# Aatricks/LightDiffusion-Next

Measured on AMD Instinct MI355X. Metric: sampler it/s (UNet steps/sec) SD1.5 1024x1024 bs=1 bf16, higher is better.
Workload: dtype bf16

## Files before the change

### include/ldx.h

```cpp
#ifndef LDX_H
#define LDX_H
#include <stdint.h>
#ifdef __cplusplus
extern "C" {
#endif

#define LDX_OK 0
#define LDX_EINVAL (-1)
#define LDX_EMISSING (-2)
#define LDX_EHIP (-3)
#define LDX_ESTATE (-4)

#define LDX_BF16 0
#define LDX_F16 1
#define LDX_F32 2

typedef struct ldx_engine ldx_engine;

typedef struct ldx_unet_config {
    int32_t compute_dtype;
    int32_t in_channels;
    int32_t out_channels;
    int32_t model_channels;
    int32_t num_levels;
// ... 33 lines not shown
    int32_t d_ff;
    int32_t num_layers;
    int32_t num_heads;
    int32_t vocab_size;
} ldx_t5_config;

typedef struct ldx_esrgan_config {
    int32_t compute_dtype;
    int32_t in_nc;
    int32_t out_nc;
    int32_t nf;
    int32_t gc;
    int32_t num_blocks;
    int32_t num_upscale;
} ldx_esrgan_config;

typedef struct ldx_flux_config {
    int32_t compute_dtype;
    int32_t in_channels;
    int32_t vec_in_dim;
    int32_t context_in_dim;
    int32_t hidden_size;
    int32_t mlp_hidden;
    int32_t num_heads;
    int32_t depth;
    int32_t depth_single;
    int32_t guidance_embed;
} ldx_flux_config;

const char* ldx_version(void);
const char* ldx_last_error(void);
int ldx_create(const ldx_unet_config* cfg, int device, ldx_engine** out);
void ldx_destroy(ldx_engine* e);
int ldx_load_tensor(ldx_engine* e, const char* key, const void* data, int dtype, const int64_t* shape, int ndim);
int ldx_set_tables(ldx_engine* e, const float* log_sigmas, int n, const float* temb, int temb_dim);
int ldx_finalize(ldx_engine* e);

int ldx_unet_denoise(ldx_engine* e, const float* x_nchw, const float* sigma, const float* ctx,
                     int B2, int h, int w, int M, float* out_nchw, void* stream);
int ldx_unet_denoise_concat(ldx_engine* e, const float* x_nchw, const float* sigma, const float* ctx, const float* c_concat, int cc_channels,
                            int B2, int h, int w, int M, float* out_nchw, void* stream);
int ldx_unet_denoise_cfg(ldx_engine* e, const float* x_nchw, float sigma, const float* ctx,
                         int B, int h, int w, int M, float* out_nchw, void* stream);
int ldx_unet_denoise_cfg_t(ldx_engine* e, const float* x_nchw, float sigma, int t_index, const float* ctx,
                           int B, int h, int w, int M, float* out_nchw, void* stream);
int ldx_unet_denoise_t(ldx_engine* e, const float* x_nchw, const float* sigma, const float* t_index, const float* ctx,
                       int B2, int h, int w, int M, float* out_nchw, void* stream);
int ldx_unet_timestep(ldx_engine* e, const float* sigma, int n, int32_t* t_out, void* stream);
int ldx_unet_context_cache(ldx_engine* e, int enable);
int ldx_unet_forward(ldx_engine* e, const float* x_nchw, const float* timesteps, const float* ctx,
                     int B2, int h, int w, int M, float* out_nchw, void* stream);
int ldx_plan_info(ldx_engine* e, int64_t* n_launches, double* flops, int64_t* arena_bytes);
int ldx_unet_cfg_share(ldx_engine* e, int enable);
int ldx_plan_flops(ldx_engine* e, double* executed, double* shared);
int ldx_profile(ldx_engine* e, int enable, int reset);
int ldx_profile_report(ldx_engine* e, char* buf, int64_t cap);
int ldx_set_graph_mode(ldx_engine* e, int enable);
int ldx_graph_stats(ldx_engine* e, int64_t* captures, int64_t* replays);
int ldx_reload_env(void);

int ldx_vae_create(const ldx_vae_config* cfg, int device, ldx_engine** out);
int ldx_vae_decode(ldx_engine* e, const float* z_nchw, int B, int h, int w, float* out_nhwc, void* stream);
int ldx_vae_encode(ldx_engine* e, const float* pixels_nhwc, int B, int H, int W, float* moments_nchw, void* stream);
int ldx_clip_create(const ldx_clip_config* cfg, int device, ldx_engine** out);
int ldx_clip_encode(ldx_engine* e, const int32_t* ids, int B, int T, int inter_layer,
                    float* out_last, float* out_inter, void* stream);
int ldx_clip_pooled(ldx_engine* e, const float* last, const int32_t* ids, int B, int T, int eos_token_id,
                    float* out_pooled, void* stream);
int ldx_clip_set_extra_embeddings(ldx_engine* e, const float* rows_host, int n);

int ldx_esrgan_create(const ldx_esrgan_config* cfg, int device, ldx_engine** out);
int ldx_esrgan_forward(ldx_engine* e, const float* pixels_nhwc, int B, int H, int W, float* out_nhwc, void* stream);
int ldx_tile_blend(const float* tile, int th, int tw, float* out, float* div, int H, int W, int C, int y0, int x0, int feather, void* stream);
int ldx_tile_finish(float* out, const float* div, int64_t n, int clamp01, void* stream);

int ldx_flux_fbcache(ldx_engine* e, float residual_diff_threshold);
int ldx_flux_fbcache_stats(ldx_engine* e, int64_t* hits, int64_t* misses);
int ldx_flux_set_fp8(ldx_engine* e, int enable);

int ldx_t5_create(const ldx_t5_config* cfg, int device, ldx_engine** out);
int ldx_t5_encode(ldx_engine* e, const int32_t* ids, int B, int L, const float* bias, float* out, void* stream);

int ldx_flux_create(const ldx_flux_config* cfg, int device, ldx_engine** out);
int ldx_flux_forward(ldx_engine* e, const float* x, const float* sigma, const float* ctx, const float* y,
                     const float* guidance, const float* pe_cos, const float* pe_sin,
                     int B, int h, int w, int Lt, int denoise, float* out, void* stream);

int ldx_sampler_step(int kind, float* x, const float* den_uncond, const float* den_cond, float* denoised_out,
                     int64_t n, float cfg, float c0, float c1, void* stream);
int ldx_bislerp_pass(const float* in, float* out, int N, int C, int H, int W, int axis, int new_len,
                     const int32_t* c1, const int32_t* c2, const float* ratios, void* stream);
int ldx_bilinear(const float* in, float* out, int planes, int hin, int win, int hout, int wout, void* stream);

int ldx_op_convert(const float* in_f32, void* out_16, int64_t n, int dtype, int to_f32, void* stream);
int ldx_op_gemm(const void* A, int lda, const void* W, int M, int N, int K, const float* bias,
                const float* rowvec, int rowvec_ld, int rows_per_batch, int geglu,
                const void* R, int ldr, void* C, int ldc, float* Cf, int ldcf, int dtype, void* stream);
int ldx_op_layernorm_mx(const void* X, int ldx, int rows, int C, float eps, const float* gamma, const float* beta,
                        void* Y8, int ldy8, void* S8, int s8_ld, int dtype, void* stream);
int ldx_op_qk_norm_rope_mx(const void* QKV, int ld, int rows, int L, int H, const float* qscale, const float* kscale, const float* cosT, const float* sinT, float eps,
                           void* Q8, void* K8, int ld8, void* SQ, void* SK, int s_ld, int dtype, void* stream);
int ldx_op_mx_vt_quant(const void* V, int ldv, int B, int H, int L, void* V8T, void* SV, int Lp, int dtype, void* stream);
int ldx_op_attention_fp8(const void* Q8, int ldq8, const void* SQ, int sq_ld, const void* K8, int ldk8, const void* SK, int sk_ld, const void* V8T, const void* SV, int Lp,
                         void* O, int ldo, void* O8, int ldo8, void* SO, int so_ld, int B, int H, int Nq, int Mk, float scale, int dtype, void* stream);
int ldx_op_attention_mx(const void* Q, int ldq, const void* K, int ldk, const void* V, int ldv, void* O8, int ldo8, void* SO, int so_ld,
                        int B, int H, int Nq, int Mk, float scale, int dtype, void* stream);
int ldx_op_mx_quant(const void* X, int ldx, int rows, int K, void* Y, int ldy, void* scales, int scales_ld, int dtype, void* stream);
int ldx_op_gemm_mx(const void* A8, int lda, const void* SA, int sa_ld, const void* W8, const void* SW, int sw_ld, int M, int N, int K,
                   const float* bias, int act, const void* R, int ldr, void* C, int ldc, float* Cf, int ldcf,
                   void* C8, int ldc8, void* SC, int sc_ld, int dtype, void* stream);
int ldx_op_gemm2(const void* A1, int lda1, const void* W1, int M1, int N1, int K1, const float* bias1, void* C1, int ldc1,
                 const void* A2, int lda2, const void* W2, int M2, int N2, int K2, const float* bias2, void* C2, int ldc2, int dtype, void* stream);
int ldx_op_gemm2_mx(const void* A1, int lda1, const void* SA1, int sa_ld1, const void* W1, const void* SW1, int sw_ld1, int M1, int N1, int K1,
                    const float* bias1, void* C1, int ldc1,
                    const void* A2, int lda2, const void* SA2, int sa_ld2, const void* W2, const void* SW2, int sw_ld2, int M2, int N2, int K2,
                    const float* bias2, void* C2, int ldc2, int dtype, void* stream);
int ldx_op_gemm_pick(int M, int N, int K, int mode, int geglu, int splitk, int f8, int c8, int ln_fold,
                     int Cin, int Hin, int Win, int Hout, int Wout, int stride, int M2, int N2, int K2,
                     int gn_hw, int gn_groups, int gn_max_chunks, int32_t* out);
int ldx_op_attn_pick(int B, int H, int Nq, int Mk, int D, int causal, int bias, int o8, int ldq, int ldk, int ldv, int ldo, int knorm_ws, int32_t* out);
int ldx_op_conv3x3(const void* X, int ldx, const void* W, int B, int Hin, int Win, int Cin, int Cout,
                   int stride, int Hout, int Wout, int resize_to_out, const float* bias,
                   const float* rowvec, int rowvec_ld, const void* R, int ldr, void* Y, int ldy,
                   int dtype, void* stream);
int ldx_op_conv3x3_skip(const void* X, int ldx, const void* X2, int ldx2, int Cin2, const void* W, int B, int H, int Wd, int Cin, int Cout,
                        const float* bias, void* Y, int ldy, int dtype, void* stream);
int ldx_op_groupnorm(const void* X, int ldx, void* Y, int ldy, int B, int HW, int C, int G, float eps, int silu,
                     const float* gamma, const float* beta, float* workspace, int dtype, void* stream);
int64_t ldx_op_groupnorm_workspace_floats(int B, int G);
int ldx_op_layernorm(const void* X, int ldx, void* Y, int ldy, int rows, int C, float eps,
                     const float* gamma, const float* beta, int dtype, void* stream);
int ldx_op_attention(const void* Q, int ldq, const void* K, int ldk, const void* V, int ldv, void* O, int ldo,
                     int B, int H, int Nq, int Mk, int D, float scale, int causal, int dtype, void* stream);
int ldx_op_xattn_block(void* H, int ldh, int64_t M, int N, int C, int heads, const float* ln_gamma, const float* ln_beta, float eps,
                       const void* Wq, const void* Wo, const float* bo, const void* K, int ldk, const void* V, int ldv, int Mk,
                       float scale, int dtype, void* stream);
int ldx_op_ff_block(void* H, int ldh, int64_t M, int C, int inner, const float* ln_gamma, const float* ln_beta, float eps,
                    const void* W1, const float* b1, const void* W2, const float* b2, int dtype, void* stream);
int ldx_op_rowgemm(const void* X, int ldx, void* Y, int ldy, int64_t M, int N, int K, const void* W, const float* bias, const void* R, int ldr,
                   int pro, const float* gamma, const float* beta, float eps, const float* partial, int nchunk, int HW, int dtype, void* stream);
int ldx_op_attention_bias(const void* Q, int ldq, const void* K, int ldk, const void* V, int ldv, void* O, int ldo,
                          int B, int H, int Nq, int Mk, int D, float scale, const float* bias, int bias_ld,
                          int64_t bias_head_stride, int dtype, void* stream);
int ldx_op_skinny(const float* x, int ldx, const void* W, const float* bias, float* out, int ldo,
                  int M, int N, int K, int in_act, int out_act, int dtype, void* stream);

#ifdef __cplusplus
}
#endif
#endif
```

### lightdiffusion-next_amd/csrc/attn_pipe.hip

```cpp
#include <stdlib.h>
#include <math.h>
#include <type_traits>
#include <utility>
#include "ldx_device.h"
#include "ldx_kernels.h"
#include "attn_pipe_common.h"

namespace ldx {

template <typename T>
__global__ __launch_bounds__(256) void attn_knorm_kernel(const AttnArgs p) {
    const int lane = threadIdx.x & 63, nblk = (p.Mk + 63) >> 6;
    const long w = (long)blockIdx.x * 4 + (threadIdx.x >> 6);
    if (w >= (long)p.B * p.H * nblk) return;
    const int blk = (int)(w % nblk), hb = (int)(w / nblk), h = hb % p.H, b = hb / p.H;
    const int key = blk * 64 + lane;
    float ss = 0.f;
    if (key < p.Mk) {
        const T* kp = (const T*)p.K + ((long)b * p.Mk + key) * p.ldk + h * p.D;
        for (int ch = 0; ch < p.D / 8; ++ch) {
            float f[8]; unpack8<T>(*(const uint4*)(kp + ch * 8), f);
#pragma unroll
            for (int e = 0; e < 8; ++e) ss = fmaf(f[e], f[e], ss);
        }
// ... 261 lines not shown
            });
        };
        if constexpr (KB) {
            if (__builtin_amdgcn_ballot_w64(ap_max2(bm0, bm1) > thr) != 0) {
                asm volatile("s_nop 15\n\ts_nop 15" ::: "memory");
                ap_for(ap_range<0, 8>(), [&](auto M) __attribute__((always_inline)) { maxblk(M, sn); });
                bm0 = bmax(0); bm1 = bmax(1);
                if (__builtin_amdgcn_ballot_w64(ap_max2(bm0, bm1) > thr) != 0) raise_reference();
            }
        } else {
            if (__builtin_amdgcn_ballot_w64(ap_max2(bm0, bm1) > thr) != 0) raise_reference();
        }
    };
    const unsigned klast = (unsigned)(nblk - 1) * kstep, vlast = (unsigned)(nblk - 1) * vstep;
    unsigned kofs = min(4u * kstep, klast), vofs = min(2u * vstep, vlast);
    for (int t = 0; t < nblk; t += 2) {
        slot(t, sA, sB, pA, pB, vfA, vfB, rsA, rsB, ap_ic<0>{}, kofs, vofs);
        kofs = min(kofs + kstep, klast); vofs = min(vofs + vstep, vlast);
        slot(t + 1, sB, sA, pB, pA, vfB, vfA, rsB, rsA, ap_ic<1>{}, kofs, vofs);
        kofs = min(kofs + kstep, klast); vofs = min(vofs + vstep, vlast);
    }
    ap_for(ap_range<0, 16>(), [&](auto J) __attribute__((always_inline)) { pv1(J, pA, vfA); });
    asm volatile("s_nop 15\n\ts_nop 15\n\ts_nop 15" ::: "memory");

#pragma unroll
    for (int qt = 0; qt < 2; ++qt) {
        const float mine = (h2 == 0) ? o[qt][1][4] : 0.f;
        auto sw = __builtin_amdgcn_permlane32_swap(__float_as_uint(mine), __float_as_uint(mine), false, false);
        const float l = __uint_as_float(sw[0]) + __uint_as_float(sw[1]);
        const float inv = (l > 0.f) ? 1.0f / l : 0.f;
        const int q = q0 + qt * 32 + l31;
#pragma unroll
        for (int dt = 0; dt < 2; ++dt)
#pragma unroll
            for (int rq = 0; rq < 4; ++rq) {
                const int d = dt * 32 + 8 * rq + 4 * h2;
                if (d < D)
                    *(uint2*)(Op + (long)q * p.ldo + d) = pack4<T>(o[qt][dt][4 * rq] * inv, o[qt][dt][4 * rq + 1] * inv, o[qt][dt][4 * rq + 2] * inv, o[qt][dt][4 * rq + 3] * inv);
            }
    }
}


void launch_attn_knorm(const AttnArgs& a, DType dt, hipStream_t s) {
    const long waves = (long)a.B * a.H * ((a.Mk + 63) / 64);
    if (dt == DT_BF16) hipLaunchKernelGGL((attn_knorm_kernel<__bf16>), dim3((unsigned)((waves + 3) / 4)), dim3(256), 0, s, a);
    else hipLaunchKernelGGL((attn_knorm_kernel<_Float16>), dim3((unsigned)((waves + 3) / 4)), dim3(256), 0, s, a);
}

template <typename T, int ABL = 0>
static void launch_attn40p(const AttnArgs& a, const AttnPick& p, hipStream_t s, float thr) {
    if (p.knorm && ABL == 0) {
        const long waves = (long)a.B * a.H * ((a.Mk + 63) / 64);
        hipLaunchKernelGGL((attn_knorm_kernel<T>), dim3((unsigned)((waves + 3) / 4)), dim3(256), 0, s, a);
        hipLaunchKernelGGL((attn40p_kernel<T, ABL, true>), dim3(p.grid), dim3(p.block), p.lds, s, a, thr);
    } else {
        hipLaunchKernelGGL((attn40p_kernel<T, ABL, false>), dim3(p.grid), dim3(p.block), p.lds, s, a, thr);
    }
}

void launch_attn_pipe(const AttnArgs& a, const AttnPick& p, DType dt, hipStream_t s) {
    const bool ov = p.thr == p.thr;
#ifdef LDX_ATTN_ABLATE
    if (const char* e = getenv("LDX_ATTN_PIPE_ABL")) {
        const float thr = ApT<__bf16>::thr;
        switch (atoi(e)) {
            case 1: launch_attn40p<__bf16, 1>(a, p, s, thr); return;
            case 2: launch_attn40p<__bf16, 2>(a, p, s, thr); return;
            case 8: launch_attn40p<__bf16, 8>(a, p, s, thr); return;
            case 16: launch_attn40p<__bf16, 16>(a, p, s, thr); return;
            case 32: launch_attn40p<__bf16, 32>(a, p, s, thr); return;
            case 9: launch_attn40p<__bf16, 9>(a, p, s, thr); return;
            case 25: launch_attn40p<__bf16, 25>(a, p, s, thr); return;
            case 27: launch_attn40p<__bf16, 27>(a, p, s, thr); return;
            case 59: launch_attn40p<__bf16, 59>(a, p, s, thr); return;
            default: break;
        }
    }
#endif
    if (dt == DT_BF16) launch_attn40p<__bf16>(a, p, s, ov ? p.thr : ApT<__bf16>::thr);
    else launch_attn40p<_Float16>(a, p, s, ov ? fminf(p.thr, ApT<_Float16>::thr) : ApT<_Float16>::thr);
}

}
```

### lightdiffusion-next_amd/csrc/attn_pipe128.hip

```cpp
#include <stdlib.h>
#include <math.h>
#include "ldx_device.h"
#include "ldx_kernels.h"
#include "attn_pipe_common.h"

namespace ldx {

template <typename T> __device__ __forceinline__ int ap128_half_a(float sa, float c, float nm, float& x, float px, float py) {
    int r;
    if constexpr (std::is_same<T, __bf16>::value) asm("v_fma_f32 %1, %2, %3, %4\n\tv_exp_f32 %1, %1\n\tv_cvt_pk_bf16_f32 %0, %5, %6" : "=&v"(r), "=&v"(x) : "v"(sa), "s"(c), "v"(nm), "v"(px), "v"(py));
    else asm("v_fma_f32 %1, %2, %3, %4\n\tv_exp_f32 %1, %1\n\tv_cvt_pk_f16_f32 %0, %5, %6" : "=&v"(r), "=&v"(x) : "v"(sa), "s"(c), "v"(nm), "v"(px), "v"(py));
    return r;
}
template <typename T> __device__ __forceinline__ void ap128_half_b(float sb, float c, float nm, float& y, float& l, int r, int ones) {
    if constexpr (std::is_same<T, __bf16>::value) asm("v_fma_f32 %0, %2, %3, %4\n\tv_exp_f32 %0, %0\n\tv_dot2_f32_bf16 %1, %5, %6, %1" : "=&v"(y), "+v"(l) : "v"(sb), "s"(c), "v"(nm), "v"(r), "s"(ones));
    else asm("v_fma_f32 %0, %2, %3, %4\n\tv_exp_f32 %0, %0\n\tv_dot2_f32_f16 %1, %5, %6, %1" : "=&v"(y), "+v"(l) : "v"(sb), "s"(c), "v"(nm), "v"(r), "s"(ones));
}
__device__ __forceinline__ void ap128_exp1(float s, float c, float nm, float& x) {
    asm("v_fma_f32 %0, %1, %2, %3\n\tv_exp_f32 %0, %0" : "=&v"(x) : "v"(s), "s"(c), "v"(nm));
}
template <typename T> __device__ __forceinline__ void ap128_sacc0(f32x16& d, ap_i32x4 a, ap_i32x4 b) {
    if constexpr (std::is_same<T, __bf16>::value) asm volatile(AP_BF16 " %0, %1, %2, 0" : "=&v"(d) : "v"(a), "a"(b));
    else asm volatile(AP_F16 " %0, %1, %2, 0" : "=&v"(d) : "v"(a), "a"(b));
}
// ... 271 lines not shown
    constexpr int EROW = 272, EROW8 = 144;
    char* ep = smem + wave * (64 * EROW);
#pragma unroll
    for (int qt = 0; qt < 2; ++qt) {
        auto sw = __builtin_amdgcn_permlane32_swap(__float_as_uint(lsum[qt]), __float_as_uint(lsum[qt]), false, false);
        const float l = __uint_as_float(sw[0]) + __uint_as_float(sw[1]);
        const float inv = (l > 0.f) ? 1.0f / l : 0.f;
        const int q = q0 + qt * 32 + l31;
        if (p.O8) {
            uint32_t sc = 0;
#pragma unroll
            for (int dt = 0; dt < 4; ++dt) {
                float v[16], amax = 0.f;
#pragma unroll
                for (int r = 0; r < 16; ++r) { v[r] = to_f32(from_f32<T>(o[qt][dt][r] * inv)); amax = fmaxf(amax, fabsf(v[r])); }
                auto am = __builtin_amdgcn_permlane32_swap(__float_as_uint(amax), __float_as_uint(amax), false, false);
                amax = fmaxf(__uint_as_float(am[0]), __uint_as_float(am[1]));
                const int e = mx_scale_e8m0(amax);
                const float is = mx_inv_scale(e);
                sc |= (uint32_t)e << (8 * dt);
#pragma unroll
                for (int rq = 0; rq < 4; ++rq)
                    *(uint32_t*)(ep + (qt * 32 + l31) * EROW8 + dt * 32 + 8 * rq + 4 * h2) = mx_pack4(v[4 * rq] * is, v[4 * rq + 1] * is, v[4 * rq + 2] * is, v[4 * rq + 3] * is);
            }
            if (h2 == 0) p.SO[(long)h * p.so_ld + (long)b * p.Nq + q] = sc;
            continue;
        }
#pragma unroll
        for (int dt = 0; dt < 4; ++dt)
#pragma unroll
            for (int rq = 0; rq < 4; ++rq)
                *(uint2*)(ep + (qt * 32 + l31) * EROW + (dt * 32 + 8 * rq + 4 * h2) * 2) = pack4<T>(o[qt][dt][4 * rq] * inv, o[qt][dt][4 * rq + 1] * inv, o[qt][dt][4 * rq + 2] * inv, o[qt][dt][4 * rq + 3] * inv);
    }
    asm volatile("s_waitcnt lgkmcnt(0)" ::: "memory");
    if (p.O8) {
        char* o8 = (char*)p.O8 + ((long)b * p.Nq + q0) * p.ldo8 + h * 128;
#pragma unroll
        for (int i = 0; i < 8; ++i) {
            const int row = i * 8 + (lane >> 3), ch = lane & 7;
            *(uint4*)(o8 + (long)row * p.ldo8 + ch * 16) = *(const uint4*)(ep + row * EROW8 + ch * 16);
        }
    } else {
#pragma unroll
        for (int i = 0; i < 16; ++i) {
            const int row = i * 4 + (lane >> 4), ch = lane & 15;
            *(uint4*)(Op + (long)(q0 + row) * p.ldo + ch * 8) = *(const uint4*)(ep + row * EROW + ch * 16);
        }
    }
}

template <typename T, int ABL = 0>
static void launch_attn128p(const AttnArgs& a, const AttnPick& p, hipStream_t s, float thr) {
    if (p.knorm && ABL == 0) {
        launch_attn_knorm(a, std::is_same<T, __bf16>::value ? DT_BF16 : DT_F16, s);
        static DevOnce once;
        set_dyn_lds(once, (const void*)attn128p_kernel<T, ABL, true>, p.lds);
        hipLaunchKernelGGL((attn128p_kernel<T, ABL, true>), dim3(p.grid), dim3(p.block), p.lds, s, a, thr);
    } else {
        static DevOnce once;
        set_dyn_lds(once, (const void*)attn128p_kernel<T, ABL, false>, p.lds);
        hipLaunchKernelGGL((attn128p_kernel<T, ABL, false>), dim3(p.grid), dim3(p.block), p.lds, s, a, thr);
    }
}

void launch_attn_pipe128(const AttnArgs& a, const AttnPick& p, DType dt, hipStream_t s) {
    const bool ov = p.thr == p.thr;
#ifdef LDX_ATTN_ABLATE
    if (const char* e = getenv("LDX_ATTN_PIPE_ABL")) {
        const float thr = ApT<__bf16>::thr;
        switch (atoi(e)) {
            case 1: launch_attn128p<__bf16, 1>(a, p, s, thr); return;
            case 2: launch_attn128p<__bf16, 2>(a, p, s, thr); return;
            case 4: launch_attn128p<__bf16, 4>(a, p, s, thr); return;
            case 8: launch_attn128p<__bf16, 8>(a, p, s, thr); return;
            case 16: launch_attn128p<__bf16, 16>(a, p, s, thr); return;
            case 32: launch_attn128p<__bf16, 32>(a, p, s, thr); return;
            case 34: launch_attn128p<__bf16, 34>(a, p, s, thr); return;
            case 24: launch_attn128p<__bf16, 24>(a, p, s, thr); return;
            case 58: launch_attn128p<__bf16, 58>(a, p, s, thr); return;
            case 62: launch_attn128p<__bf16, 62>(a, p, s, thr); return;
            default: break;
        }
    }
#endif
    if (dt == DT_BF16) launch_attn128p<__bf16>(a, p, s, ov ? p.thr : ApT<__bf16>::thr);
    else launch_attn128p<_Float16>(a, p, s, ov ? fminf(p.thr, ApT<_Float16>::thr) : ApT<_Float16>::thr);
}

}
```

### lightdiffusion-next_amd/csrc/capi.cpp

```cpp
#include <cstring>
#include <mutex>
#include <new>

#include "engine.h"

using namespace ldx;

struct ldx_engine { Engine* impl; };

#define GUARD_BEGIN try {
#define GUARD_END                                                                  \
    }                                                                              \
    catch (const std::bad_alloc&) { set_error("out of host memory"); return LDX_EINVAL; } \
    catch (const std::exception& ex) { set_error(std::string("internal error: ") + ex.what()); return LDX_EINVAL; }

static int check_device(int device) {
    int n = 0;
    if (hipGetDeviceCount(&n) != hipSuccess || n <= 0) { set_error("no HIP device available (libldx has no CPU fallback)"); return LDX_EHIP; }
    if (device < 0 || device >= n) { set_error("device ordinal out of range"); return LDX_EINVAL; }
    return LDX_OK;
}
static inline DType dtype_of(int d) { return d == LDX_F16 ? DT_F16 : DT_BF16; }
static int check_launch(const char* what) {
    hipError_t e = hipGetLastError();
// ... 223 lines not shown
}
int ldx_unet_denoise_cfg(ldx_engine* e, const float* x, float sigma, const float* ctx, int B, int h, int w, int M, float* out, void* stream) {
    GUARD_BEGIN
    if (!e) { set_error("null engine"); return LDX_EINVAL; }
    if (e->impl->kind != KIND_UNET) { set_error("ldx_unet_denoise_cfg: not a UNet engine"); return LDX_ESTATE; }
    return e->impl->run_cfg(x, sigma, ctx, B, h, w, M, out, (hipStream_t)stream);
    GUARD_END
}
int ldx_unet_denoise_cfg_t(ldx_engine* e, const float* x, float sigma, int t_index, const float* ctx, int B, int h, int w, int M, float* out, void* stream) {
    GUARD_BEGIN
    if (!e) { set_error("null engine"); return LDX_EINVAL; }
    if (e->impl->kind != KIND_UNET) { set_error("ldx_unet_denoise_cfg_t: not a UNet engine"); return LDX_ESTATE; }
    return e->impl->run_cfg(x, sigma, ctx, B, h, w, M, out, (hipStream_t)stream, t_index < 0 ? -1 : t_index);
    GUARD_END
}
int ldx_unet_denoise_t(ldx_engine* e, const float* x, const float* sigma, const float* t_index, const float* ctx, int B2, int h, int w, int M, float* out, void* stream) {
    GUARD_BEGIN
    if (!e) { set_error("null engine"); return LDX_EINVAL; }
    if (e->impl->kind != KIND_UNET) { set_error("ldx_unet_denoise_t: not a UNet engine"); return LDX_ESTATE; }
    if (!t_index) { set_error("ldx_unet_denoise_t: t_index is null (use ldx_unet_denoise)"); return LDX_EINVAL; }
    return e->impl->run(x, sigma, ctx, B2, h, w, M, out, true, (hipStream_t)stream, 0, nullptr, 0, t_index);
    GUARD_END
}
int ldx_unet_timestep(ldx_engine* e, const float* sigma, int n, int32_t* t_out, void* stream) {
    GUARD_BEGIN
    if (!e) { set_error("null engine"); return LDX_EINVAL; }
    return e->impl->timestep_lookup(sigma, n, (int*)t_out, (hipStream_t)stream);
    GUARD_END
}
int ldx_unet_forward(ldx_engine* e, const float* x, const float* t, const float* ctx, int B2, int h, int w, int M, float* out, void* stream) {
    GUARD_BEGIN
    if (!e) { set_error("null engine"); return LDX_EINVAL; }
    if (e->impl->kind != KIND_UNET) { set_error("ldx_unet_forward: not a UNet engine"); return LDX_ESTATE; }
    return e->impl->run(x, t, ctx, B2, h, w, M, out, false, (hipStream_t)stream);
    GUARD_END
}
int ldx_plan_info(ldx_engine* e, int64_t* n_launches, double* flops, int64_t* arena_bytes) {
    if (!e) { set_error("null engine"); return LDX_EINVAL; }
    if (n_launches) *n_launches = e->impl->n_launches();
    if (flops) *flops = e->impl->algorithmic_flops();
    if (arena_bytes) *arena_bytes = (int64_t)e->impl->cur.arena_cap;
    return LDX_OK;
}
int ldx_plan_flops(ldx_engine* e, double* executed, double* shared) {
    if (!e) { set_error("null engine"); return LDX_EINVAL; }
    if (executed) *executed = e->impl->steady_flops();
    if (shared) *shared = e->impl->cur.flops_shared;
    return LDX_OK;
}
int ldx_unet_cfg_share(ldx_engine* e, int enable) {
    if (!e) { set_error("null engine"); return LDX_EINVAL; }
    if (e->impl->kind != KIND_UNET) { set_error("ldx_unet_cfg_share: not a UNet engine"); return LDX_ESTATE; }
    e->impl->cfg_share = enable < 0 ? 0 : (enable > 2 ? 2 : enable);
    return LDX_OK;
}
int ldx_profile(ldx_engine* e, int enable, int reset) {
    if (!e) { set_error("null engine"); return LDX_EINVAL; }
    e->impl->profiling = enable != 0;
    e->impl->prof_detail = enable == 2;
    if (reset) e->impl->prof.clear();
    return LDX_OK;
}
int ldx_profile_report(ldx_engine* e, char* buf, int64_t cap) {
    if (!e || !buf || cap <= 0) { set_error("ldx_profile_report: bad argument"); return LDX_EINVAL; }
    const std::string s = e->impl->profile_json();
    if ((int64_t)s.size() + 1 > cap) { set_error("ldx_profile_report: buffer too small"); return LDX_EINVAL; }
    memcpy(buf, s.c_str(), s.size() + 1);
    return LDX_OK;
}
int ldx_set_graph_mode(ldx_engine* e, int enable) {
    if (!e) { set_error("null engine"); return LDX_EINVAL; }
    e->impl->graph_mode = enable != 0;
    return LDX_OK;
}
int ldx_unet_context_cache(ldx_engine* e, int enable) {
    if (!e) { set_error("null engine"); return LDX_EINVAL; }
    if (e->impl->kind != KIND_UNET) { set_error("ldx_unet_context_cache: not a UNet engine"); return LDX_ESTATE; }
    return e->impl->set_context_cache(enable);
}
int ldx_reload_env(void) {
    reload_dispatch_env();
    return LDX_OK;
}
int ldx_graph_stats(ldx_engine* e, int64_t* captures, int64_t* replays) {
    if (!e || !captures || !replays) { set_error("ldx_graph_stats: bad argument"); return LDX_EINVAL; }
    *captures = e->impl->n_graph_captures; *replays = e->impl->n_graph_replays;
    return LDX_OK;
}

int ldx_sampler_step(int kind, float* x, const float* du, const float* dc, float* dout, int64_t n, float cfg, float c0, float c1, void* stream) {
    if (!x || !du || !dc || n < 0 || (kind < 0 || kind > 3)) { set_error("ldx_sampler_step: bad argument"); return LDX_EINVAL; }
    if (kind == 2 && !dout) { set_error("ldx_sampler_step: kind 2 (CFG combine only) needs denoised_out"); return LDX_EINVAL; }
    if (kind == 0 && c0 == 0.f) { set_error("ldx_sampler_step: kind 0 (Euler) divides by c0 = sigma_hat, which must be non-zero"); return LDX_EINVAL; }
    StepArgs a{x, du, dc, dout, (size_t)n, cfg, kind, c0, c1};
    launch_sampler_step(a, (hipStream_t)stream);
    return check_launch("ldx_sampler_step");
}
int ldx_bislerp_pass(const float* in, float* out, int N, int C, int H, int W, int axis, int new_len,
                     const int32_t* c1, const int32_t* c2, const float* ratios, void* stream) {
    if (!in || !out || !c1 || !c2 || !ratios || N <= 0 || C <= 0 || C > 16 || H <= 0 || W <= 0 || new_len <= 0 || (axis != 0 && axis != 1)) {
        set_error("ldx_bislerp_pass: bad argument (C <= 16, axis 0|1)"); return LDX_EINVAL; }
    launch_bislerp_pass(in, out, N, C, H, W, axis, new_len, (const int*)c1, (const int*)c2, ratios, (hipStream_t)stream);
    return check_launch("ldx_bislerp_pass");
}
int ldx_vae_encode(ldx_engine* e, const float* pixels_nhwc, int B, int H, int W, float* moments_nchw, void* stream) {
    GUARD_BEGIN
// ... 206 lines not shown
    launch_groupnorm(a, dtype_of(dtype), (hipStream_t)stream);
    return check_launch("ldx_op_groupnorm");
}
int ldx_op_layernorm(const void* X, int ldx_, void* Y, int ldy, int rows, int C, float eps, const float* gamma, const float* beta, int dtype, void* stream) {
    if (!X || !Y || !gamma || !beta || C % 8 || C > 4096) { set_error("ldx_op_layernorm: bad argument (C % 8, C <= 4096)"); return LDX_EINVAL; }
    LayerNormArgs a{X, ldx_, Y, ldy, rows, C, eps, gamma, beta};
    launch_layernorm(a, dtype_of(dtype), (hipStream_t)stream);
    return check_launch("ldx_op_layernorm");
}
int ldx_op_attention(const void* Q, int ldq, const void* K, int ldk, const void* V, int ldv, void* O, int ldo, int B, int H, int Nq, int Mk, int D,
                     float scale, int causal, int dtype, void* stream) {
    if (!Q || !K || !V || !O || D % 8 || (D > 160 && D != 512) || D <= 0 || ldq % 8 || ldk % 8 || ldv % 8 || ldo % 4 || Mk <= 0) { set_error("ldx_op_attention: bad argument (D % 8, D <= 160 or D == 512)"); return LDX_EINVAL; }
    AttnArgs a{Q, ldq, K, ldk, V, ldv, O, ldo, B, H, Nq, Mk, D, scale, causal, nullptr, 0, 0};
    const AttnPick p = attn_pick(a);
    if (D == 512 && p.family != AF_ATTN512) { set_error("ldx_op_attention: D = 512 without a mask only (attn512.hip)"); return LDX_EINVAL; }
    if (p.nsplit_want > 1) {
        a.nsplit = p.nsplit_want;
        a.split_ws = op_workspace(attn512_ws_floats(a, a.nsplit));
        if (!a.split_ws) { set_error("attention split workspace allocation failed"); return LDX_EHIP; }
    }
    if (attn_pipe_ok(a)) a.knorm_ws = op_workspace((size_t)B * H * ((Mk + 63) / 64));
    launch_attention(a, dtype_of(dtype), (hipStream_t)stream);
    return check_launch("ldx_op_attention");
}
int ldx_op_xattn_block(void* H, int ldh, int64_t M, int N, int C, int heads, const float* ln_gamma, const float* ln_beta, float eps,
                       const void* Wq, const void* Wo, const float* bo, const void* K, int ldk, const void* V, int ldv, int Mk,
                       float scale, int dtype, void* stream) {
    XAttnArgs a{};
    a.H = H; a.ldh = ldh; a.M = (long)M; a.N = N; a.C = C; a.heads = heads; a.ln_g = ln_gamma; a.ln_b = ln_beta; a.eps = eps;
    a.Wq = Wq; a.Wo = Wo; a.bo = bo; a.K = K; a.ldk = ldk; a.V = V; a.ldv = ldv; a.Mk = Mk; a.scale = scale;
    if (!H || !ln_gamma || !ln_beta || !Wq || !Wo || !K || !V || M <= 0 || N <= 0 || ldh < C || !xattn_block_ok(a)) {
        set_error("ldx_op_xattn_block: shape not taken by the fused kernel (C = 320, 8 heads, Mk <= 80, N % 128 == 0, M % N == 0)"); return LDX_EINVAL; }
    launch_xattn_block(a, dtype_of(dtype), (hipStream_t)stream);
    return check_launch("ldx_op_xattn_block");
}
int ldx_op_ff_block(void* H, int ldh, int64_t M, int C, int inner, const float* ln_gamma, const float* ln_beta, float eps,
                    const void* W1, const float* b1, const void* W2, const float* b2, int dtype, void* stream) {
    FFBlockArgs a{};
    a.H = H; a.ldh = ldh; a.M = (long)M; a.C = C; a.inner = inner; a.ln_g = ln_gamma; a.ln_b = ln_beta; a.eps = eps; a.W1 = W1; a.b1 = b1; a.W2 = W2; a.b2 = b2;
    if (!H || !ln_gamma || !ln_beta || !W1 || !b1 || !W2 || M <= 0 || ldh < C || !ff_block_ok(a)) {
        set_error("ldx_op_ff_block: shape not taken by the fused kernel (C = 320, inner = 1280)"); return LDX_EINVAL; }
    launch_ff_block(a, dtype_of(dtype), (hipStream_t)stream);
    return check_launch("ldx_op_ff_block");
}
int ldx_op_rowgemm(const void* X, int ldx_, void* Y, int ldy, int64_t M, int N, int K, const void* W, const float* bias, const void* R, int ldr,
                   int pro, const float* gamma, const float* beta, float eps, const float* partial, int nchunk, int HW, int dtype, void* stream) {
    RowGemmArgs a{};
    a.X = X; a.ldx = ldx_; a.Y = Y; a.ldy = ldy; a.M = (long)M; a.N = N; a.K = K; a.W = W; a.bias = bias; a.R = R; a.ldr = ldr;
    a.pro = pro; a.g = gamma; a.b = beta; a.eps = eps; a.partial = partial; a.nchunk = nchunk; a.HW = HW; a.G = 32;
    if (!X || !Y || !W || ldx_ < K || ldy < N || !rowgemm_ok(a)) { set_error("ldx_op_rowgemm: shape not taken (K = 320 or 640, N a multiple of K, pro 0..2, GroupNorm: HW % (40960 / K) == 0, nchunk <= 256)"); return LDX_EINVAL; }
    launch_rowgemm(a, dtype_of(dtype), (hipStream_t)stream);
    return check_launch("ldx_op_rowgemm");
}
int ldx_op_attention_bias(const void* Q, int ldq, const void* K, int ldk, const void* V, int ldv, void* O, int ldo, int B, int H, int Nq, int Mk, int D,
                          float scale, const float* bias, int bias_ld, int64_t bias_head_stride, int dtype, void* stream) {
    if (!Q || !K || !V || !O || !bias || D % 8 || D > 160 || D <= 0 || ldq % 8 || ldk % 8 || ldv % 8 || ldo % 4 || Mk <= 0 || bias_ld % 4 ||
        bias_ld < ((Mk + 63) / 64) * 64 || bias_head_stride % 4) {
        set_error("ldx_op_attention_bias: bad argument (bias_ld >= Mk rounded up to 64, multiples of 4)"); return LDX_EINVAL; }
    AttnArgs a{Q, ldq, K, ldk, V, ldv, O, ldo, B, H, Nq, Mk, D, scale, 0, bias, bias_ld, (long)bias_head_stride};
    launch_attention(a, dtype_of(dtype), (hipStream_t)stream);
    return check_launch("ldx_op_attention_bias");
}
int ldx_op_skinny(const float* x, int ldx_, const void* W, const float* bias, float* out, int ldo, int M, int N, int K, int in_act, int out_act, int dtype, void* stream) {
    if (!x || !W || !out || K % 8) { set_error("ldx_op_skinny: bad argument"); return LDX_EINVAL; }
    SkinnyArgs a{x, ldx_, W, bias, out, ldo, M, N, K, in_act, out_act};
    launch_skinny(a, dtype_of(dtype), (hipStream_t)stream);
    return check_launch("ldx_op_skinny");
}

}
```

### lightdiffusion-next_amd/csrc/engine.cpp

```cpp
#include "engine.h"

#include <algorithm>
#include <cmath>
#include <cstdio>
#include <cstring>
#include <thread>

namespace ldx {

thread_local std::string g_last_error;
void set_error(const std::string& s) { g_last_error = s; }
int launch_status() {
    const hipError_t e = hipGetLastError();
    if (e == hipSuccess) return LDX_OK;
    set_error(std::string("kernel launch: ") + hipGetErrorString(e));
    return LDX_EHIP;
}

#define HIP_OK(expr)                                                                         \
    do {                                                                                     \
        hipError_t _e = (expr);                                                              \
        if (_e != hipSuccess) {                                                              \
            set_error(std::string(#expr) + ": " + hipGetErrorString(_e));                    \
            return LDX_EHIP;                                                                 \
// ... 547 lines not shown
        GemmArgs& g = cur.ops[i - 1].g;
        GroupNormArgs& n = cur.ops[i].gn;
        if (g.C != n.X || g.ldc != n.ldx || g.N != n.C || (long)g.M != (long)n.B * n.HW) continue;
        const int nchunk = gemm_gn_fuse(g, n.HW, n.G, gn_ws_rows);
        if (!nchunk) continue;
        g.gn_partial = n.partial;
        n.stats_chunks = nchunk;
        cur.ops[i].bytes = 2.0 * 2.0 * (double)n.B * n.HW * n.C;
        snprintf(cur.ops[i].klabel, sizeof(cur.ops[i].klabel), "gn_apply(fused stats)");
    }
}
bool Engine::rowblock_fills_chip(long workgroups) const {
    static const long min_wg = getenv("LDX_ROWBLOCK_MINWG") ? atol(getenv("LDX_ROWBLOCK_MINWG")) : 192;
    static const long min_wg_prefix = getenv("LDX_ROWBLOCK_MINWG_PREFIX") ? atol(getenv("LDX_ROWBLOCK_MINWG_PREFIX")) : 96;
    return workgroups >= (rowblock_prefix ? (min_wg_prefix < min_wg ? min_wg_prefix : min_wg) : min_wg);
}
bool Engine::op_rowgemm(const char* name, Act X, const LinearW& w, Act Y, Act R, int pro, const NormW* nw) {
    RowGemmArgs a{};
    a.X = ptr(X); a.ldx = X.ld; a.Y = ptr(Y); a.ldy = Y.ld; a.M = X.rows; a.N = w.N; a.K = w.K; a.W = w.w; a.bias = w.b;
    a.R = R.valid ? ptr(R) : nullptr; a.ldr = R.ld; a.pro = pro; a.eps = 1e-5f;
    if (nw) { a.g = nw->g; a.b = nw->b; }
    static const long plain640_maxm = getenv("LDX_ROWGEMM_PLAIN640_MAXM") ? atol(getenv("LDX_ROWGEMM_PLAIN640_MAXM")) : 16384;
    if (pro == 0 && a.K == 640 && a.M > plain640_maxm) return false;
    if (!w.w || !rowgemm_ok(a) || !rowblock_fills_chip((a.M + 128 * 320 / a.K - 1) / (128 * 320 / a.K) * (a.K / 320))) return false;
    Op o{}; o.kind = OP_ROWGEMM; o.name = name; o.rg = a;
    o.flops = 2.0 * a.M * (double)a.N * a.K;
    o.bytes = 2.0 * ((double)a.M * a.K + (double)a.N * a.K + (double)a.M * a.N * (R.valid ? 2 : 1));
    snprintf(o.klabel, sizeof(o.klabel), "rowgemm<%s,%d>", dt == DT_BF16 ? "bf16" : "f16", pro);
    cur.ops.push_back(o);
    cur.flops += o.flops;
    return true;
}
void Engine::fuse_gn_rowgemm() {
    for (size_t i = 0; i + 1 < cur.ops.size(); ++i) {
        rowblock_prefix = i < cur.prefix_end;
        if (cur.ops[i].kind != OP_GN || cur.ops[i + 1].kind != OP_GEMM) continue;
        const GroupNormArgs& n = cur.ops[i].gn;
        const GemmArgs& g = cur.ops[i + 1].g;
        if (n.silu || n.stats_chunks <= 0 || n.stats_chunks > GN_NCHUNK || n.G != 32 || g.A != n.Y || g.lda != n.ldy || g.mode != 0 || g.K != n.C || g.geglu || g.ln_c1 ||
            g.f8 || g.C8 || g.Cf || g.rowvec || g.splitk > 1 || g.gate || g.R2 || g.act || g.oscale != 0.f || g.gn_partial || g.dup_rows || (long)g.M != (long)n.B * n.HW || !g.C) continue;
        RowGemmArgs a{};
        a.X = n.X; a.ldx = n.ldx; a.Y = g.C; a.ldy = g.ldc; a.M = g.M; a.N = g.N; a.K = g.K; a.W = g.W; a.bias = g.bias; a.R = g.R; a.ldr = g.ldr;
        a.pro = 2; a.g = n.gamma; a.b = n.beta; a.eps = n.eps; a.partial = n.partial; a.nchunk = n.stats_chunks; a.HW = n.HW; a.G = n.G;
        if (!rowgemm_ok(a) || !rowblock_fills_chip((a.M + 128 * 320 / a.K - 1) / (128 * 320 / a.K) * (a.K / 320))) continue;
        Op o{}; o.kind = OP_ROWGEMM; o.name = cur.ops[i + 1].name; o.rg = a;
        o.flops = cur.ops[i + 1].flops; o.bytes = cur.ops[i + 1].bytes;
        snprintf(o.klabel, sizeof(o.klabel), "rowgemm<%s,2>", dt == DT_BF16 ? "bf16" : "f16");
        cur.ops[i] = o;
        cur.ops.erase(cur.ops.begin() + (long)i + 1);
        if (i + 1 < cur.prefix_end) --cur.prefix_end;
    }
    rowblock_prefix = false;
}
void Engine::op_ln(const char* name, Act X, Act Y, const NormW& n) {
    Op o{}; o.kind = OP_LN; o.name = name;
    LayerNormArgs& l = o.ln;
    l.X = ptr(X); l.ldx = X.ld; l.Y = ptr(Y); l.ldy = Y.ld; l.rows = X.rows; l.C = n.C; l.eps = 1e-5f; l.gamma = n.g; l.beta = n.b;
    o.bytes = 2.0 * 2.0 * (double)X.rows * n.C;
    snprintf(o.klabel, sizeof(o.klabel), "ln_kernel");
    cur.ops.push_back(o);
}
void Engine::op_attn(const char* name, const void* Q, int ldq, const void* K, int ldk, const void* V, int ldv, Act O, int B, int H, int Nq, int Mk, int D) {
    Op o{}; o.kind = OP_ATTN; o.name = name;
    AttnArgs& a = o.at;
    a.Q = Q; a.ldq = ldq; a.K = K; a.ldk = ldk; a.V = V; a.ldv = ldv; a.O = ptr(O); a.ldo = O.ld;
    a.B = B; a.H = H; a.Nq = Nq; a.Mk = Mk; a.D = D; a.scale = 1.0f / std::sqrt((float)D); a.causal = 0;
    if (attn_pipe_ok(a)) {
        const size_t off = a_alloc((size_t)B * H * ((Mk + 63) / 64) * 4); a.knorm_ws = (float*)((uintptr_t)cur.arena + off); a_free(off);
    }
    const AttnPick p = attn_pick(a);
    if (p.nsplit_want > 1) {
        a.nsplit = p.nsplit_want;
        const size_t off = a_alloc(attn512_ws_floats(a, a.nsplit) * 4); a.split_ws = (float*)((uintptr_t)cur.arena + off); a_free(off);
    }
    o.flops = 4.0 * B * H * (double)Nq * Mk * D;
    o.bytes = 2.0 * (double)B * H * D * (2.0 * Nq + 2.0 * Mk);
    {
        static const char* const fmt[] = {"attn_kernel<%s,%d,%d,%d>", "attn32_kernel<%s,%d,144,192,%d>", "attn32ap_kernel<%s,144,192,%d>", "attn32g_kernel<%s,%d,%d,1,%d,%d>",
                                          "attn40p_kernel<%s>", "attn128p_kernel<%s>", "attn512_kernel<%s>"};
        const int n = snprintf(o.klabel, sizeof(o.klabel), fmt[p.family], dt == DT_BF16 ? "bf16" : "f16", p.targ[0], p.targ[1], p.targ[2], (int)p.kpf);
        if (p.family == AF_ATTN512) snprintf(o.klabel + n, sizeof(o.klabel) - n, "x%d", a.nsplit);
        else snprintf(o.klabel + n, sizeof(o.klabel) - n, "%s", Nq == Mk ? "self" : "cross");
    }
    cur.ops.push_back(o);
    cur.flops += o.flops;
}

void Engine::op_dup(const Act& a, int rows) {
    Op o{}; o.kind = OP_DUP; o.name = "cfg.dup";
    o.p0 = ptr(a); o.p1 = cur.arena ? (char*)ptr(a) + (size_t)rows * a.ld * 2 : nullptr; o.i0 = rows; o.i1 = a.C; o.i2 = a.ld;
    o.bytes = 2.0 * 2.0 * (double)rows * a.C;
    snprintf(o.klabel, sizeof(o.klabel), "dup_rows");
    cur.ops.push_back(o);
}

void Engine::dup_second_half(const DupReq& d) {
    static const bool copy_only = getenv("LDX_CFG_SHARE_COPY") && atoi(getenv("LDX_CFG_SHARE_COPY")) != 0;
    if (!copy_only && d.producer < cur.ops.size()) {
        Op& o = cur.ops[d.producer];
        if (o.kind == OP_GEMM && o.g.C == ptr(d.a) && o.g.ldc == d.a.ld && o.g.M == d.rows && !o.g.geglu && !o.g.C8) { o.g.dup_rows = d.rows; return; }
        if (o.kind == OP_ROWGEMM && o.rg.Y == ptr(d.a) && o.rg.ldy == d.a.ld && o.rg.M == d.rows) { o.rg.dup_rows = d.rows; return; }
    }
    op_dup(d.a, d.rows);
}

Act Engine::new_act(int rows, int C) {
// ... 84 lines not shown
        xa.scale = q_prescale() ? 1.0f / 1.44269504088896340736f : 1.0f / std::sqrt((float)D);
        if (!fold && !b.q2.b && xattn_block_ok(xa) && rowblock_fills_chip((M + 127) / 128)) {
            Op o{}; o.kind = OP_XATTN; o.name = "xf.xattn2"; o.xa = xa;
            o.flops = 2.0 * 2.0 * M * (double)C * C + 4.0 * B * heads * (double)(H * W) * Mc * D;
            o.bytes = 2.0 * 2.0 * (double)M * C;
            snprintf(o.klabel, sizeof(o.klabel), "xattn_block<%s>", dt == DT_BF16 ? "bf16" : "f16");
            cur.ops.push_back(o);
            cur.flops += o.flops;
            release(a);
        } else {
            Act q = new_act(M, C);
            static const bool x2 = !(getenv("LDX_ROWGEMM_X2") && atoi(getenv("LDX_ROWGEMM_X2")) == 0);
            if (!x2 || fold || b.q2.b || !op_rowgemm("xf.ln2+q2", h, b.q2, q, Act{}, 1, &b.ln2))
                ln_gemm("xf.ln2", "xf.q2", b.ln2, fold ? b.q2_f : b.q2, b.c1_q2, q, false);
            op_attn("xf.attn2", ptr(q), C, kvb, kv_total, kvb + (size_t)C * 2, kv_total, a, B, heads, H * W, Mc, D);
            if (q_prescale()) cur.ops.back().at.scale = 1.0f / 1.44269504088896340736f;
            release(q);
            if (!x2 || !op_rowgemm("xf.o2", a, b.o2, h, h, 0, nullptr))
                op_gemm("xf.o2", a, b.o2, h, h);
            release(a);
        }
        FFBlockArgs fa{};
        fa.H = ptr(h); fa.ldh = h.ld; fa.M = M; fa.C = C; fa.inner = 4 * C; fa.ln_g = b.ln3.g; fa.ln_b = b.ln3.b; fa.eps = 1e-5f;
        fa.W1 = b.ff1.w; fa.b1 = b.ff1.b; fa.W2 = b.ff2.w; fa.b2 = b.ff2.b;
        if (!fold && ff_block_ok(fa) && rowblock_fills_chip((M + 127) / 128)) {
            Op o{}; o.kind = OP_FFBLOCK; o.name = "xf.ffblock"; o.fb = fa;
            o.flops = 2.0 * M * (double)C * (8.0 * C) + 2.0 * M * (double)C * (4.0 * C);
            o.bytes = 2.0 * 2.0 * (double)M * C;
            snprintf(o.klabel, sizeof(o.klabel), "ff_block<%s>", dt == DT_BF16 ? "bf16" : "f16");
            cur.ops.push_back(o);
            cur.flops += o.flops;
        } else {
            Act f = new_act(M, 4 * C);
            ln_gemm("xf.ln3", "xf.ff1", b.ln3, fold ? b.ff1_f : b.ff1, b.c1_ff1, f, true);
            op_gemm("xf.ff2", f, b.ff2, h, h);
            release(f);
        }
    }
    if (n.valid) release(n);
    static const bool po = !(getenv("LDX_ROWGEMM_PO") && atoi(getenv("LDX_ROWGEMM_PO")) == 0);
    if (!po || !op_rowgemm("xf.proj_out", h, x.proj_out, OUT, X, 0, nullptr))
        op_gemm("xf.proj_out", h, x.proj_out, OUT, X);
    release(h);
}

int Engine::share_for(int B2, int h, int w, int xB, bool denoise, bool concat) const {
    static const long share_minrows = getenv("LDX_CFG_SHARE_MINROWS") ? atol(getenv("LDX_CFG_SHARE_MINROWS")) : 8192;
    if (!cfg_share || !denoise || concat || xB <= 0 || B2 != 2 * xB || (cfg_share == 1 && (long)xB * h * w < share_minrows)) return 0;
    for (auto& blk : in_blocks) if (blk.has_xf) return xB;
    return 0;
}

int Engine::plan(int B2, int h, int w, int Mc, int share) {
    return build_plan(PlanKey{B2, h, w, Mc, share}, [&]() -> int {
        const int mc = cfg.model_channels, ted = 4 * mc;
        const size_t o_temb = a_alloc((size_t)B2 * mc * 4), o_e1 = a_alloc((size_t)B2 * ted * 4), o_e2 = a_alloc((size_t)B2 * ted * 4);
        const size_t o_emb = a_alloc((size_t)B2 * emb_total * 4);
        cur.gn_ws_off = a_alloc(gn_ws_bytes(B2, (long)h * w));
        const size_t o_eps = a_alloc((size_t)B2 * h * w * cfg.out_channels * 4);
        auto f32p = [&](size_t off) { return cur.arena ? (float*)((char*)cur.arena + off) : (float*)nullptr; };
        cur.d_temb_out = f32p(o_temb); cur.d_e1 = f32p(o_e1); cur.d_e2 = f32p(o_e2); cur.d_emb_all = f32p(o_emb); cur.d_eps = f32p(o_eps);

        struct Skip { Act act; int H, W; };
        std::vector<int> Hs{h}, Ws{w};
        for (int l = 1; l < cfg.num_levels; ++l) { Hs.push_back((Hs.back() + 1) / 2); Ws.push_back((Ws.back() + 1) / 2); }
        std::vector<int> in_ch{mc}, in_lv{0};
        { int c = mc; for (int l = 0; l < cfg.num_levels; ++l) { for (int r = 0; r < cfg.num_res_blocks[l]; ++r) { c = mc * cfg.channel_mult[l]; in_ch.push_back(c); in_lv.push_back(l); }
              if (l != cfg.num_levels - 1) { in_ch.push_back(c); in_lv.push_back(l + 1); } } }
        const int n_skips = (int)in_ch.size();
        std::vector<int> out_hch(n_skips);
        { int c = in_ch.back(); int k = 0;
          for (int l = cfg.num_levels - 1; l >= 0; --l) for (int i = 0; i <= cfg.num_res_blocks[l]; ++i) { out_hch[k++] = c; c = mc * cfg.channel_mult[l]; } }
        std::vector<Act> cat(n_skips);
        for (int k = 0; k < n_skips; ++k) {
            const int s = n_skips - 1 - k, lv = in_lv[s];
            cat[k] = new_act(B2 * Hs[lv] * Ws[lv], out_hch[k] + in_ch[s]);
        }
        auto skip_view = [&](int s) { const int k = n_skips - 1 - s; return view(cat[k], out_hch[k], in_ch[s]); };

        Op po{}; po.kind = OP_PREP; po.name = "prep"; cur.ops.push_back(po);
        Act xin = new_act(B2 * h * w, 64);
        cur.prep_xc_off = xin.off;
        Act ctx16 = new_act(B2 * Mc, cfg.context_dim);
        { Op o{}; o.kind = OP_CVT; o.name = "ctx.cvt"; o.cvt_out = ptr(ctx16); o.cvt_n = (size_t)B2 * Mc * cfg.context_dim; o.ctx_only = true; cur.ops.push_back(o); }
        if (!d_emb_table) {
            { Op o{}; o.kind = OP_SKINNY; o.name = "time_embed.0"; o.sk = SkinnyArgs{cur.d_temb_out, mc, te0.w, te0.b, cur.d_e1, ted, B2, ted, mc, 0, 1}; cur.ops.push_back(o); }
            { Op o{}; o.kind = OP_SKINNY; o.name = "time_embed.2"; o.sk = SkinnyArgs{cur.d_e1, ted, te2.w, te2.b, cur.d_e2, ted, B2, ted, ted, 0, 1}; cur.ops.push_back(o); }
            { Op o{}; o.kind = OP_SKINNY; o.name = "emb_layers"; o.sk = SkinnyArgs{cur.d_e2, ted, emb_all.w, emb_all.b, cur.d_emb_all, emb_total, B2, emb_total, ted, 0, 0}; cur.ops.push_back(o); }
            cur.flops += 2.0 * B2 * ((double)ted * mc + (double)ted * ted + (double)emb_total * ted);
        }
        Act kvall = new_act(B2 * Mc, kv_total);
        cur.kv_all_off = kvall.off;
        op_gemm("xf.kv2_all", ctx16, kv_all, kvall, Act{});
        cur.ops.back().ctx_only = true;

        int lv = 0, s = 0;
        Act hcur = skip_view(0);
        int Bp = share > 0 ? share : B2;
        std::vector<DupReq> pend;
        op_conv("conv_in", xin, Bp, h, w, 64, conv_in, 1, h, w, hcur, Act{});
        cur.flops -= 2.0 * Bp * h * w * (double)mc * 9.0 * (64 - cfg.in_channels);
        release(xin);
        if (Bp != B2) pend.push_back({hcur, Bp * h * w, cur.ops.size() - 1});
        for (auto& blk : in_blocks) {
            ++s;
            Act dst = skip_view(s);
            if (blk.has_down) {
// ... 33 lines not shown
                emit_res(mid_res0, hcur, dst, B2, Hs[lv], Ws[lv]);
            }
        }
        int k = 0;
        Act final_h{};
        for (auto& blk : out_blocks) {
            const int sidx = n_skips - 1 - k; (void)sidx;
            const bool last = (k == n_skips - 1);
            const int Hc = Hs[lv], Wc = Ws[lv], Mrows = B2 * Hc * Wc;
            const int co = blk.res.Cout;
            int nsub = 1 + (blk.has_xf ? 1 : 0) + (blk.has_up ? 1 : 0);
            auto target = [&](bool is_final_sub, int rows) -> Act {
                if (is_final_sub && !last) return view(cat[k + 1], 0, out_hch[k + 1]);
                return new_act(rows, co);
            };
            int sub = 0;
            Act x = cat[k];
            Act r_out = target(++sub == nsub, Mrows);
            emit_res(blk.res, x, r_out, B2, Hc, Wc);
            release(cat[k]);
            x = r_out;
            if (blk.has_xf) {
                Act x_out = target(++sub == nsub, Mrows);
                emit_xf(blk.xf, x, x_out, B2, Hc, Wc, ctx16, Mc);
                release(x);
                x = x_out;
            }
            if (blk.has_up) {
                const int Hn = Hs[lv - 1], Wn = Ws[lv - 1];
                Act u_out = target(++sub == nsub, B2 * Hn * Wn);
                op_conv("up", x, B2, Hc, Wc, co, blk.up, 1, Hn, Wn, u_out, Act{});
                release(x);
                x = u_out; --lv;
            }
            final_h = x;
            ++k;
        }
        {
            const int Mrows = B2 * h * w;
            Act t = new_act(Mrows, mc);
            op_gn("out.gn", final_h, t, B2, h * w, out_gn, 1e-5f, true);
            release(final_h);
            op_conv("out.conv", t, B2, h, w, mc, conv_out, 1, h, w, Act{}, Act{}, nullptr, 0, cur.d_eps, cfg.out_channels);
            release(t);
        }
        { Op o{}; o.kind = OP_FINISH; o.name = "finish"; cur.ops.push_back(o); }
        release(ctx16); release(kvall);
        if (share > 0) {
            for (size_t i = 0; i < cur.prefix_end && i < cur.ops.size(); ++i) if (!cur.ops[i].ctx_only) cur.flops_shared += cur.ops[i].flops;
            cur.flops_shared -= 2.0 * share * h * w * (double)mc * 9.0 * (64 - cfg.in_channels);
        }
        fuse_gn_stats();
        fuse_gn_rowgemm();
        return LDX_OK;
    });
}

int Engine::build_emb_table() {
    static const bool off = getenv("LDX_EMB_TABLE") && atoi(getenv("LDX_EMB_TABLE")) == 0;
    if (off || d_emb_table || !d_temb || n_sigmas <= 0 || emb_total <= 0 || emb_total % 4) return LDX_OK;
    const int mc = cfg.model_channels, ted = 4 * mc, n = n_sigmas;
    float *e1 = nullptr, *e2 = nullptr, *tab = nullptr;
    auto fail = [&](hipError_t err, const char* what) {
        if (e1) (void)hipFree(e1);
        if (e2) (void)hipFree(e2);
        if (tab) (void)hipFree(tab);
        set_error(std::string(what) + ": " + hipGetErrorString(err));
        return LDX_EHIP;
    };
    hipError_t err;
    if ((err = hipMalloc((void**)&e1, (size_t)n * ted * 4)) != hipSuccess) return fail(err, "build_emb_table: hipMalloc");
    if ((err = hipMalloc((void**)&e2, (size_t)n * ted * 4)) != hipSuccess) return fail(err, "build_emb_table: hipMalloc");
    if ((err = hipMalloc((void**)&tab, (size_t)n * emb_total * 4)) != hipSuccess) return fail(err, "build_emb_table: hipMalloc");
    launch_skinny(SkinnyArgs{d_temb, mc, te0.w, te0.b, e1, ted, n, ted, mc, 0, 1}, dt, nullptr);
    launch_skinny(SkinnyArgs{e1, ted, te2.w, te2.b, e2, ted, n, ted, ted, 0, 1}, dt, nullptr);
    launch_skinny(SkinnyArgs{e2, ted, emb_all.w, emb_all.b, tab, emb_total, n, emb_total, ted, 0, 0}, dt, nullptr);
    if ((err = hipStreamSynchronize(nullptr)) != hipSuccess) return fail(err, "build_emb_table: hipStreamSynchronize");
    if ((err = hipGetLastError()) != hipSuccess) return fail(err, "build_emb_table: kernel launch");
    (void)hipFree(e1); (void)hipFree(e2);
    dev_allocs.push_back(tab);
    d_emb_table = tab;
    weight_bytes += (size_t)n * emb_total * 4;
    return LDX_OK;
}

double Engine::steady_flops() const {
    double f = cur.flops;
    if (ctx_cache) for (const Op& o : cur.ops) if (o.ctx_only) f -= o.flops;
    return f;
}
double Engine::algorithmic_flops() const { return steady_flops() + cur.flops_shared; }

void Plan::release() {
    if (arena) (void)hipFree(arena);
    if (graph_exec) (void)hipGraphExecDestroy(graph_exec);
    arena = nullptr; graph_exec = nullptr;
}

int Engine::build_plan(const PlanKey& key, const std::function<int()>& emit, bool zero_arena) {
    auto reset = [&] {
        free_list.clear(); live.clear(); arena_top = 0; arena_peak = 0; rowblock_prefix = false;
        cur.ops.clear(); cur.flops = 0; cur.flops_shared = 0; cur.prefix_end = 0;
    };
    cur.key = PlanKey{};
    reset();
    void* const arena = cur.arena;
// ... 144 lines not shown
                else if (o.kind == OP_GN) snprintf(sh, sizeof(sh), " B%d HW%d C%d", o.gn.B, o.gn.HW, o.gn.C);
                else if (o.kind == OP_ROWGEMM) snprintf(sh, sizeof(sh), " M%ld N%d K%d", o.rg.M, o.rg.N, o.rg.K);
                else if (o.kind == OP_XATTN) snprintf(sh, sizeof(sh), " M%ld C%d", (long)o.xa.M, o.xa.C);
                else if (o.kind == OP_FFBLOCK) snprintf(sh, sizeof(sh), " M%ld C%d", (long)o.fb.M, o.fb.C);
                else if (o.kind == OP_LN) snprintf(sh, sizeof(sh), " R%d C%d", o.ln.rows, o.ln.C);
                else if (o.kind == OP_MXQ) snprintf(sh, sizeof(sh), " R%d K%d", o.mq.rows, o.mq.K);
                else if (o.kind == OP_GEMM2) snprintf(sh, sizeof(sh), " M%d+%d N%d K%d", o.g.M, o.g2.M, o.g.N, o.g.K);
                key += sh;
            }
            ProfEntry& pe = prof[key];
            pe.count += 1; pe.ms += ms; pe.flops += o.flops; pe.bytes += o.bytes;
        }
    }
    return LDX_OK;
}

int Engine::run_cfg(const float* x, float sigma, const float* ctx, int B, int h, int w, int Mc, float* out, hipStream_t st, int t_index) {
    if (B <= 0) { set_error("ldx_unet_denoise_cfg: bad argument"); return LDX_EINVAL; }
    if (t_index >= n_sigmas) { set_error("ldx_unet_denoise_cfg_t: t_index outside the sigma table"); return LDX_EINVAL; }
    HIP_OK(hipSetDevice(device));
    if (sigma_cfg_cap < 2 * B) {
        HIP_OK(hipStreamSynchronize(st));
        if (d_sigma_cfg) (void)hipFree(d_sigma_cfg);
        d_sigma_cfg = nullptr; sigma_cfg_cap = 0;
        HIP_OK(hipMalloc((void**)&d_sigma_cfg, sizeof(float) * 4 * B));
        sigma_cfg_cap = 2 * B;
    }
    float* d_t = d_sigma_cfg + sigma_cfg_cap;
    if (t_index >= 0) launch_fill2_f32(d_sigma_cfg, sigma, d_t, (float)t_index, 2 * B, st);
    else launch_fill_f32(d_sigma_cfg, sigma, 2 * B, st);
    return run(x, d_sigma_cfg, ctx, 2 * B, h, w, Mc, out, true, st, B, nullptr, 0, t_index >= 0 ? d_t : nullptr);
}
int Engine::timestep_lookup(const float* sigma_dev, int n, int* out_dev, hipStream_t st) {
    if (kind != KIND_UNET || !d_log_sigmas) { set_error("ldx_unet_timestep: needs a UNet engine with its sigma table (ldx_set_tables)"); return LDX_ESTATE; }
    if (!sigma_dev || !out_dev || n < 0) { set_error("ldx_unet_timestep: bad argument"); return LDX_EINVAL; }
    HIP_OK(hipSetDevice(device));
    launch_timestep(sigma_dev, d_log_sigmas, n_sigmas, n, out_dev, st);
    HIP_OK(hipGetLastError());
    return LDX_OK;
}

int Engine::run(const float* x, const float* sigma_or_t, const float* ctx, int B2, int h, int w, int Mc, float* out, bool denoise, hipStream_t st, int xB,
                const float* c_concat, int cc_channels, const float* t_idx) {
    if (!denoise) t_idx = nullptr;
    if (c_concat && (cc_channels <= 0 || cc_channels >= cfg.in_channels || (denoise && cfg.in_channels - cc_channels != cfg.out_channels))) {
        set_error("ldx_unet_denoise_concat: c_concat channels must leave the latent's channels (in_channels - cc_channels == out_channels)"); return LDX_EINVAL;
    }
    if (!c_concat) cc_channels = 0;
    if (xB < 0 || (xB > 0 && B2 % xB != 0)) { set_error("ldx_unet_*: the batch of x must divide the evaluation batch"); return LDX_EINVAL; }
    if (!finalized) { set_error("ldx_unet_*: engine not finalized"); return LDX_ESTATE; }
    if (!x || !sigma_or_t || !ctx || !out || B2 <= 0 || h <= 0 || w <= 0 || Mc <= 0) { set_error("ldx_unet_*: bad argument"); return LDX_EINVAL; }
    HIP_OK(hipSetDevice(device));
    const int share = share_for(B2, h, w, xB, denoise, c_concat != nullptr);
    if (int rc = select_plan(PlanKey{B2, h, w, Mc, share}, st, [&] { return plan(B2, h, w, Mc, share); })) return rc;
    bind = Bindings{};
    bind.x = x; bind.s = sigma_or_t; bind.ctx = ctx; bind.out = out; bind.den = denoise; bind.xB = xB; bind.cc = c_concat; bind.ccn = cc_channels; bind.t = t_idx;
    bind.ctxc = ctx_cache;
    if (bind.ctxc && !(cur.kv_ptr == ctx && cur.kv_epoch == ctx_epoch && cur.kv_stream == st)) {
        const bool pg = prof_graph; prof_graph = false;
        const int rc = exec_ops(st, 0, (size_t)-1, 2);
        prof_graph = pg;
        if (rc) return rc;
        cur.kv_ptr = ctx; cur.kv_epoch = ctx_epoch; cur.kv_stream = st;
    }
    const bool same = cur.graph_b == bind;
    if (!same) cur.graph_valid = false;
    if (graph_mode && cur.graph_valid && same) {
        HIP_OK(hipGraphLaunch(cur.graph_exec, st));
        ++n_graph_replays;
        return LDX_OK;
    }
    const bool use_graph = graph_mode && cur.warm && same;
    cur.graph_b = bind; cur.warm = true;
    hipStream_t ls = st;
    if (use_graph) {
        if (cur.graph_exec) { (void)hipGraphExecDestroy(cur.graph_exec); cur.graph_exec = nullptr; }
        if (!cap_stream) HIP_OK(hipStreamCreateWithFlags(&cap_stream, hipStreamNonBlocking));
        HIP_OK(hipStreamSynchronize(st));
        HIP_OK(hipStreamBeginCapture(cap_stream, hipStreamCaptureModeThreadLocal));
        ls = cap_stream;
    }
    prof_graph = use_graph;
    { int rc = exec_ops(ls, 0, (size_t)-1, bind.ctxc ? 1 : 0); if (rc) return rc; }
    if (use_graph) {
        hipGraph_t g = nullptr;
        HIP_OK(hipStreamEndCapture(cap_stream, &g));
        HIP_OK(hipGraphInstantiate(&cur.graph_exec, g, nullptr, nullptr, 0));
        (void)hipGraphDestroy(g);
        cur.graph_valid = true;
        ++n_graph_captures;
        HIP_OK(hipGraphLaunch(cur.graph_exec, st));
    }
    return launch_status();
}

std::string Engine::profile_json() const {
    std::string s = "{";
    bool first = true;
    char buf[256];
    for (auto& kv : prof) {
        snprintf(buf, sizeof(buf), "%s\"%s\": {\"count\": %ld, \"ms\": %.6f, \"flops\": %.6e, \"bytes\": %.6e}", first ? "" : ", ",
                 kv.first.c_str(), kv.second.count, kv.second.ms, kv.second.flops, kv.second.bytes);
        s += buf; first = false;
    }
    return s + "}";
}

int64_t Engine::n_launches() const {
    int64_t n = 0;
    for (const Op& o : cur.ops) {
        if (ctx_cache && o.ctx_only) continue;
        if (o.kind == OP_GN) n += o.gn.stats_chunks > GN_NCHUNK ? 2 : (o.gn.stats_chunks > 0 ? 1 : 2);
        else if (o.kind == OP_GEMM) n += gemm_pick(o.g).launches;
        else if (o.kind == OP_GEMM2) n += gemm_pick(o.g, &o.g2).launches;
        else if (o.kind == OP_ATTN) n += attn_pick(o.at).launches;
        else n += 1;
    }
    return n;
}

}
```

### lightdiffusion-next_amd/csrc/engine.h

```cpp
#pragma once
#include <functional>
#include <initializer_list>
#include <map>
#include <string>
#include <unordered_map>
#include <utility>
#include <vector>

#include "../../include/ldx.h"
#include "ldx_kernels.h"

namespace ldx {

extern thread_local std::string g_last_error;
void set_error(const std::string& s);
int launch_status();

struct HostTensor {
    int dtype = LDX_F32;
    std::vector<int64_t> shape;
    std::vector<uint8_t> data;
    size_t numel = 0;
    float at(size_t i) const;
};

struct LinearW { void* w = nullptr; float* b = nullptr; int N = 0, K = 0;
                 void* w8 = nullptr; uint32_t* sw = nullptr; };
struct NormW { float* g = nullptr; float* b = nullptr; int C = 0; };
struct ResW { NormW gn1, gn2; LinearW conv1, conv2, skip; bool has_skip = false; bool fused_skip = false;  int Cin = 0, Cout = 0; int emb_off = 0;
              float eps = 1e-5f; bool has_emb = true; };
struct XfBlockW { NormW ln1, ln2, ln3; LinearW qkv, o1, q2, kv2, o2, ff1, ff2; LinearW qkv_f, q2_f, ff1_f;  int kv_off = 0;
    bool ln_fold = false; float *c1_qkv = nullptr, *c1_q2 = nullptr, *c1_ff1 = nullptr; };
struct XfW { NormW gn; LinearW proj_in, proj_out; std::vector<XfBlockW> blocks; int C = 0, depth = 0; };
struct BlockW { bool has_res = false, has_xf = false, has_down = false, has_up = false; ResW res; XfW xf; LinearW down, up; int skip_ch = 0; };

struct Act { bool valid = false; bool owned = false; size_t off = 0; int rows = 0, C = 0, ld = 0, col = 0; };

enum OpKind { OP_PREP, OP_CVT, OP_SKINNY, OP_GEMM, OP_GN, OP_LN, OP_ATTN, OP_FINISH,
              OP_VAEPREP, OP_SOFTMAX, OP_CLAMP, OP_EMBED, OP_CVT_OUT,
              OP_PIXPREP, OP_MOMENTS, OP_COPY_OUT,
              OP_FX_PATCH, OP_FX_TEMB, OP_FX_SILU, OP_FX_ROPE, OP_FX_UNPATCH, OP_FX_CVT_CTX, OP_FX_SKINNY_Y, OP_FX_SKINNY_G, OP_MXQ, OP_GEMM2, OP_XATTN, OP_FFBLOCK, OP_ROWGEMM, OP_ATTN_MX, OP_MXVT, OP_DUP };
enum EngineKind { KIND_UNET = 0, KIND_VAE = 1, KIND_CLIP = 2, KIND_FLUX = 3, KIND_T5 = 4, KIND_ESRGAN = 5 };
struct Op {
    OpKind kind; const char* name;
    GemmArgs g; GemmArgs g2; GroupNormArgs gn; LayerNormArgs ln; AttnArgs at; SkinnyArgs sk; QkRopeArgs rp; MxQuantArgs mq; XAttnArgs xa; FFBlockArgs fb; RowGemmArgs rg; AttnMxArgs am; MxVtArgs vt;
    void* cvt_out; size_t cvt_n;
    bool ctx_only = false;
    const void* p0; void* p1; int i0, i1, i2, i3; float f0, f1;
    double flops; double bytes; char klabel[48];
};
struct ProfEntry { long count = 0; double ms = 0, flops = 0, bytes = 0; };

struct PlanKey {
    int B = 0, h = 0, w = 0, m = 0, share = 0;
    bool operator==(const PlanKey& o) const { return B == o.B && h == o.h && w == o.w && m == o.m && share == o.share; }
    bool operator!=(const PlanKey& o) const { return !(*this == o); }
};

struct Bindings {
    const float *x = nullptr, *s = nullptr, *ctx = nullptr; float* out = nullptr; bool den = false; int xB = 0;
    const float* cc = nullptr; int ccn = 0;
    const float* t = nullptr;
    bool ctxc = false;
    const int* ids = nullptr; float* out2 = nullptr; const float* bias = nullptr;
    const float *y = nullptr, *guid = nullptr, *pe_cos = nullptr, *pe_sin = nullptr;
    bool operator==(const Bindings& o) const {
        return x == o.x && s == o.s && ctx == o.ctx && out == o.out && den == o.den && xB == o.xB && cc == o.cc && ccn == o.ccn && t == o.t &&
               ctxc == o.ctxc && ids == o.ids && out2 == o.out2 && bias == o.bias && y == o.y && guid == o.guid && pe_cos == o.pe_cos && pe_sin == o.pe_sin;
    }
};

struct Plan {
    PlanKey key;
    std::vector<Op> ops;
    double flops = 0;
    double flops_shared = 0;
    size_t prefix_end = 0;
    void* arena = nullptr;
    size_t arena_cap = 0, arena_peak_dry = 0;
    size_t gn_ws_off = 0;
    size_t prep_xc_off = 0, kv_all_off = 0;
    float *d_temb_out = nullptr, *d_e1 = nullptr, *d_e2 = nullptr, *d_emb_all = nullptr, *d_eps = nullptr;
    const void* kv_ptr = nullptr; uint64_t kv_epoch = 0;
    hipStream_t kv_stream = nullptr;
    hipGraphExec_t graph_exec = nullptr;
    bool graph_valid = false, warm = false;
    Bindings graph_b;
    float *fx_temb = nullptr, *fx_gemb = nullptr, *fx_h1 = nullptr, *fx_vec = nullptr, *fx_svec = nullptr, *fx_mod = nullptr, *fx_tok = nullptr;
    void *fb_s0 = nullptr, *fb_s1 = nullptr, *fb_x = nullptr; float *fb_first = nullptr, *fb_res = nullptr, *fb_part = nullptr;
    int fb_B = 0, fb_L = 0, fb_Lt = 0, fb_C = 0; size_t fb_a_end = 0, fb_b_end = 0;
    void release();
};

struct EmbSrc { const HostTensor* w; const HostTensor* b; int n; };

struct VaeAttnW { NormW norm; LinearW q, k, v, proj; LinearW qkv;  };
struct ClipLayerW { NormW ln1, ln2; LinearW qkv, out, fc1, fc2; };
struct RdbW { LinearW c[5]; };
struct T5LayerW { NormW ln1, ln2; LinearW qkv, o, wi, wo; };
struct FluxStreamW { LinearW qkv, proj, mlp0, mlp2; float* qs = nullptr; float* ks = nullptr; int mod_off = 0; };
struct FluxDoubleW { FluxStreamW img, txt; };
struct FluxSingleW { LinearW lin1_qkv, lin1_mlp, lin2; float* qs = nullptr; float* ks = nullptr; int mod_off = 0; };

class Engine {
public:
    Engine(const ldx_unet_config& c, int dev);
    Engine(const ldx_vae_config& c, int dev);
    Engine(const ldx_clip_config& c, int dev);
// ... 5 lines not shown
    int finalize_esrgan();
    int plan_esrgan(int B, int H, int W);
    int run_esrgan(const float* px, int B, int H, int W, float* out, hipStream_t st);
    ldx_t5_config tcfg{};
    std::vector<T5LayerW> t5_layers; NormW t5_final_ln; float* t5_tok = nullptr;
    int finalize_t5();
    int plan_t5(int B, int L);
    int run_t5(const int* ids, int B, int L, const float* bias, float* out, hipStream_t st);
    ldx_flux_config fcfg{};
    int finalize_flux();
    float fb_threshold = 0.f; bool fb_have_first = false, fb_have_res = false; float fb_prev_t = 0.f; bool fb_prev_valid = false;
    long fb_hits = 0, fb_misses = 0;
    void fb_reset() { fb_have_first = fb_have_res = false; fb_prev_valid = false; }
    bool fx_fp8 = false;
    bool fx_fp8_attn = false;
    bool mx_quantize_weight(LinearW& w);
    int plan_flux(int B, int h, int w, int Lt);
    int run_flux(const float* x, const float* sigma, const float* ctx, const float* y, const float* guidance,
                 const float* pe_cos, const float* pe_sin, int B, int h, int w, int Lt, bool denoise, float* out, hipStream_t st);
    EngineKind kind = KIND_UNET;
    ldx_vae_config vcfg{};
    ldx_clip_config ccfg{};
    int finalize_vae();
    int finalize_clip();
    int plan_vae(int B, int h, int w);
    int plan_clip(int B, int T, int inter);
    int run_vae(const float* z, int B, int h, int w, float* out_nhwc, hipStream_t st);
    int plan_vae_encode(int B, int H, int W);
    int run_vae_encode(const float* px, int B, int H, int W, float* moments, hipStream_t st);
    int run_clip(const int* ids, int B, int T, int inter_layer, float* out_last, float* out_inter, hipStream_t st);
    int set_clip_extra(const float* rows_host, int n);
    ~Engine();
    int validate() const;
    int load_tensor(const char* key, const void* data, int dtype, const int64_t* shape, int ndim);
    int set_tables(const float* ls, int n, const float* temb, int dim);
    int finalize();
    int run(const float* x, const float* sigma_or_t, const float* ctx, int B2, int h, int w, int Mc, float* out, bool denoise, hipStream_t st, int xB = 0,
            const float* c_concat = nullptr, int cc_channels = 0, const float* t_idx = nullptr);
    int clip_pooled(const float* last, const int* ids, int B, int T, int eos_id, float* out, hipStream_t st);
    int run_cfg(const float* x, float sigma, const float* ctx, int B, int h, int w, int Mc, float* out, hipStream_t st, int t_index = -1);
    int timestep_lookup(const float* sigma_dev, int n, int* out_dev, hipStream_t st);
    float* d_sigma_cfg = nullptr; int sigma_cfg_cap = 0;
    float* d_emb_table = nullptr;
    int build_emb_table();
    bool ctx_cache = false; uint64_t ctx_epoch = 1;
    int set_context_cache(int enable) { ctx_cache = enable != 0; ++ctx_epoch; return LDX_OK; }
    double algorithmic_flops() const;
    double steady_flops() const;
    unsigned* d_sk_count = nullptr;
    unsigned* sk_counters();
    int plan(int B2, int h, int w, int Mc, int share = 0);
    int share_for(int B2, int h, int w, int xB, bool denoise, bool concat) const;
    int cfg_share = 1;
    int64_t n_launches() const;
    int64_t n_graph_captures = 0, n_graph_replays = 0;
    bool profiling = false, prof_detail = false;
    std::map<std::string, ProfEntry> prof;
    std::string profile_json() const;

    ldx_unet_config cfg;
    int device;
    DType dt;
    bool finalized = false;
    bool graph_mode = false;
    size_t weight_bytes = 0;
    Plan cur;

private:
    std::unordered_map<std::string, HostTensor> host;
    std::string missing;
    std::vector<void*> dev_allocs;
    const HostTensor* get(const std::string& key, std::initializer_list<int64_t> shape);
    void* upload16(size_t rows, size_t cols, const std::function<float(size_t, size_t)>& getter);
    float* upload32(size_t n, const std::function<float(size_t)>& getter);
    bool mk_linear(const std::string& pre, int N, int K, bool bias, LinearW& out, bool conv1x1 = false);
    bool mk_conv3(const std::string& pre, int Cout, int Cin, int CinPad, LinearW& out);
    bool mk_norm(const std::string& pre, int C, NormW& out);
    bool mk_ln_folded(int N, int K, const std::function<float(size_t, size_t)>& W, const std::function<float(size_t)>& bias,
                      const std::string& norm_pre, LinearW& out, float*& c1);
    bool mk_res(const std::string& pre, int Cin, int Cout, ResW& r);
    bool mk_xf(const std::string& pre, int C, int depth, XfW& x);

    int exec_ops(hipStream_t ls, size_t op_begin = 0, size_t op_end = (size_t)-1, int ctx_sel = 0);
    int gn_ws_rows = 256;
    size_t gn_ws_bytes(int B, long HWmax) { gn_ws_rows = (int)gn_workspace_rows(HWmax); return (size_t)B * (gn_ws_rows + GN_FOLD) * 32 * 2 * 4; }
    size_t ws_alloc(size_t bytes);
    void fuse_gn_stats();
    void fuse_gn_rowgemm();
    bool op_rowgemm(const char* name, Act X, const LinearW& w, Act Y, Act R, int pro, const NormW* nw);
    Bindings bind;
    std::vector<std::vector<ResW>> vae_up; std::vector<LinearW> vae_upconv; std::vector<bool> vae_has_up;
    ResW vae_mid1, vae_mid2; VaeAttnW vae_attn; NormW vae_norm_out; float* vae_pq = nullptr;
    bool vae_has_enc = false;
    std::vector<std::vector<ResW>> enc_down; std::vector<LinearW> enc_downconv;
    ResW enc_mid1, enc_mid2; VaeAttnW enc_attn; NormW enc_norm_out; LinearW enc_conv_in, enc_conv_out; float* enc_qc = nullptr;
    bool mk_vae_attn(const std::string& pre, int C, VaeAttnW& a);
    std::vector<FluxDoubleW> fx_double; std::vector<FluxSingleW> fx_single;
    LinearW fx_img_in, fx_txt_in, fx_time0, fx_time1, fx_vec0, fx_vec1, fx_gd0, fx_gd1, fx_mod_all, fx_final;
    int fx_mod_total = 0, fx_final_mod_off = 0;
    std::vector<EmbSrc> fx_mod_srcs;
    std::vector<ClipLayerW> clip_layers; NormW clip_final_ln; float* clip_tok = nullptr; float* clip_pos = nullptr;
    float* clip_extra = nullptr; int clip_extra_n = 0, clip_extra_cap = 0;
    float* clip_proj = nullptr;
    LinearW te0, te2, conv_in, conv_out, emb_all;
    NormW out_gn;
    std::vector<BlockW> in_blocks, out_blocks;
    bool has_middle = false, mid_has_xf = false;
    ResW mid_res0, mid_res1;
    XfW mid_xf;
    int emb_total = 0;
    std::vector<EmbSrc> emb_srcs;
    struct KvSrc { const HostTensor* k; const HostTensor* v; int C; };
    std::vector<KvSrc> kv_srcs; int kv_total = 0; LinearW kv_all;
    float* d_log_sigmas = nullptr; float* d_temb = nullptr; int n_sigmas = 0;

    std::vector<std::pair<size_t, size_t>> free_list;
    std::map<size_t, size_t> live;
    size_t arena_top = 0, arena_peak = 0;
    bool rowblock_prefix = false;
    bool rowblock_fills_chip(long workgroups) const;
    int build_plan(const PlanKey& key, const std::function<int()>& emit, bool zero_arena = false);
    int select_plan(const PlanKey& key, hipStream_t st, const std::function<int()>& replan, bool* switched = nullptr);
    size_t a_alloc(size_t bytes);
    void a_free(size_t off);
    void* ptr(const Act& a) const { return (void*)((uintptr_t)cur.arena + a.off + (size_t)a.col * 2); }
    Act new_act(int rows, int C);
    Act view(const Act& base, int col, int C);
    void release(const Act& a);
    void op_gemm(const char* name, Act A, const LinearW& w, Act C, Act R, bool geglu = false, const float* rowvec = nullptr, int rv_ld = 0, int rpb = 0);
    void op_conv(const char* name, Act X, int B, int Hin, int Win, int Cin, const LinearW& w, int stride, int Hout, int Wout,
                 Act Y, Act R, const float* rowvec = nullptr, int rv_ld = 0, float* Cf = nullptr, int ldcf = 0);
    void op_gn(const char* name, Act X, Act Y, int B, int HW, const NormW& n, float eps, bool silu);
    void op_ln(const char* name, Act X, Act Y, const NormW& n);
    void op_attn(const char* name, const void* Q, int ldq, const void* K, int ldk, const void* V, int ldv, Act O, int B, int H, int Nq, int Mk, int D);
    void emit_res(const ResW& r, Act X, Act OUT, int B, int H, int W);
    void emit_vae_attn(const VaeAttnW& a, Act X, Act OUT, int B, int H, int W);
    bool mk_vae_res(const std::string& pre, int Cin, int Cout, ResW& r);
    struct DupReq { Act a; int rows; size_t producer; };
    void emit_xf(const XfW& x, Act X, Act OUT, int B, int H, int W, Act ctx16, int Mc, int Bshare = 0, const std::vector<DupReq>* dups = nullptr);
    void op_dup(const Act& a, int rows);
    void dup_second_half(const DupReq& d);
// ... 11 lines not shown
```

### lightdiffusion-next_amd/csrc/ff_block.hip

```cpp
#include <hip/hip_runtime.h>
#include <stdint.h>
#include <stdlib.h>
#include "ldx_device.h"
#include "ldx_kernels.h"
#include "rowblock_store.h"

namespace ldx {

constexpr int FB_C = 320, FB_I = 1280, FB_BM = 128, FB_CH = 128, FB_NCH = FB_I / FB_CH;
constexpr int FB_AROW = FB_C * 2 + 16;
constexpr int FB_GROW = FB_CH * 2 + 16;
constexpr int FB_ABYTES = FB_BM * FB_AROW, FB_GBYTES = FB_BM * FB_GROW;
constexpr int FB_LDS = FB_ABYTES + 2 * FB_GBYTES + 2 * FB_C * 4;

template <typename T>
__global__ __launch_bounds__(512, 1) void ff_block_kernel(const FFBlockArgs p) {
    extern __shared__ __attribute__((aligned(16))) char smem[];
    using V8 = typename Vec<T>::v8;
    char* sA = smem;
    char* sGb = smem + FB_ABYTES;
    float* sG = (float*)(smem + FB_ABYTES + 2 * FB_GBYTES);
    float* sBt = sG + FB_C;
    const int tid = threadIdx.x, lane = tid & 63;
    const int wave = __builtin_amdgcn_readfirstlane(tid >> 6);
// ... 96 lines not shown
            const int brow = (i0 >> 5) * 64 + (i0 & 31) + 4 * g4;
            const float4 bv = *(const float4*)(p.b1 + brow), bg = *(const float4*)(p.b1 + brow + 32);
#pragma unroll
            for (int qt = 0; qt < 8; ++qt) {
                const float v0 = (tv[qt][0] + bv.x) * gelu_erf_f(tg[qt][0] + bg.x), v1 = (tv[qt][1] + bv.y) * gelu_erf_f(tg[qt][1] + bg.y);
                const float v2 = (tv[qt][2] + bv.z) * gelu_erf_f(tg[qt][2] + bg.z), v3 = (tv[qt][3] + bv.w) * gelu_erf_f(tg[qt][3] + bg.w);
                *(uint2*)(sGc + (16 * qt + l15) * FB_GROW + (wave * 16 + 4 * g4) * 2) = pack4<T>(v0, v1, v2, v3);
            }
        }
        __syncthreads();
        w2_load(ch, 1, w2f); w2_load(ch, 2, w2f); w2_load(ch, 3, w2f);
        if (ch + 1 < FB_NCH) {
            const T *wv, *wg;
            w1_rows(ch + 1, wv, wg);
#pragma unroll
            for (int ks = 0; ks < PD; ++ks) { w1[ks][0] = *(const uint4*)(wv + ks * 32); w1[ks][1] = *(const uint4*)(wg + ks * 32); }
        }
#pragma unroll
        for (int ks = 0; ks < 4; ++ks) {
            V8 gf[8];
#pragma unroll
            for (int qt = 0; qt < 8; ++qt) gf[qt] = as_v8<T>(*(const uint4*)(sGc + (16 * qt + l15) * FB_GROW + (ks * 32 + g4 * 8) * 2));
#pragma unroll
            for (int t = 0; t < 3; ++t) {
                const V8 w8 = as_v8<T>(w2f[ks][t]);
#pragma unroll
                for (int qt = 0; qt < 8; ++qt) y[t][qt] = mfma16(w8, gf[qt], y[t][qt]);
            }
            __builtin_amdgcn_sched_barrier(0);
        }
    }

    uint2 rr[3][8];
#pragma unroll
    for (int t = 0; t < 3; ++t)
#pragma unroll
        for (int qt = 0; qt < 8; ++qt) {
            const long m = m0 + 16 * qt + l15;
            const int nl = 16 * t + 4 * g4;
            rr[t][qt] = (m < p.M && nl < 40) ? *(const uint2*)(Hp + m * p.ldh + wave * 40 + nl) : make_uint2(0u, 0u);
        }
#pragma unroll
    for (int t = 0; t < 3; ++t) {
        const int nl = 16 * t + 4 * g4;
        const int n = wave * 40 + (nl < 40 ? nl : 0);
        const float4 bo = p.b2 ? *(const float4*)(p.b2 + n) : make_float4(0.f, 0.f, 0.f, 0.f);
#pragma unroll
        for (int qt = 0; qt < 8; ++qt) {
            float r4[4];
            unpack4<T>(rr[t][qt], r4);
            rr[t][qt] = pack4<T>(y[t][qt][0] + bo.x + r4[0], y[t][qt][1] + bo.y + r4[1], y[t][qt][2] + bo.z + r4[2], y[t][qt][3] + bo.w + r4[3]);
        }
    }
    __syncthreads();
    rb_store_rows<T, 8>(Hp, p.ldh, m0, p.M, 0, wave, l15, g4, tid, rr, sGb);
}

bool ff_block_ok(const FFBlockArgs& a) {
    static const bool off = getenv("LDX_FF_FUSE") && atoi(getenv("LDX_FF_FUSE")) == 0;
    return !off && a.C == FB_C && a.inner == FB_I && a.M > 0 && a.ldh % 8 == 0 && a.b1 != nullptr;
}
template <typename T>
static void launch_ff_t(const FFBlockArgs& a, hipStream_t s) {
    static DevOnce once;
    set_dyn_lds(once, (const void*)ff_block_kernel<T>, FB_LDS);
    hipLaunchKernelGGL((ff_block_kernel<T>), dim3((unsigned)((a.M + FB_BM - 1) / FB_BM)), dim3(512), FB_LDS, s, a);
}
void launch_ff_block(const FFBlockArgs& a, DType dt, hipStream_t s) {
    if (dt == DT_BF16) launch_ff_t<__bf16>(a, s); else launch_ff_t<_Float16>(a, s);
}

}
```

### lightdiffusion-next_amd/csrc/ldx_kernels.h

```cpp
#pragma once
#include <hip/hip_runtime.h>
#include <stdint.h>

namespace ldx {

enum DType : int { DT_BF16 = 0, DT_F16 = 1 };

struct DevOnce { unsigned long long mask = 0; };
inline void set_dyn_lds(DevOnce& once, const void* fn, int bytes) {
    int dev = 0;
    (void)hipGetDevice(&dev);
    const unsigned long long bit = 1ull << (dev & 63);
    if (__atomic_load_n(&once.mask, __ATOMIC_RELAXED) & bit) return;
    (void)hipFuncSetAttribute(fn, hipFuncAttributeMaxDynamicSharedMemorySize, bytes);
    __atomic_fetch_or(&once.mask, bit, __ATOMIC_RELAXED);
}

struct GemmArgs {
    const void* A;  int lda;
    const void* W;
    int M, N, K;
    int mode;
    int Cin, Hin, Win;
    int Hv, Wv;
// ... 17 lines not shown
    int splitk; float* ws;
    unsigned* sk_count;
    float* gn_partial; int gn_cpg, gn_G, gn_hw, gn_nchunk;
    long dup_rows;
    int ep_general;
};
int gemm_gn_fuse(GemmArgs& a, int HW, int G, int max_chunks);
bool gemm_gn_fuse_enabled();
void launch_gemm(const GemmArgs& a, DType dt, hipStream_t s);
void launch_gemm2(const GemmArgs& a, const GemmArgs& b, DType dt, hipStream_t s);
int gemm_choose_splitk(int M, int N, int K, bool geglu);
enum GemmFamily : int { GF_TILE = 0, GF_TILE2, GF_PP, GF_PP2, GF_RING, GF_CONV_PATCH, GF_TILE_MX, GF_TILE2_MX, GF_PP_MX, GF_PP2_MX };
enum GemmReduce : int { RED_NONE = 0, RED_LAUNCH, RED_LAUNCH_GN, RED_IN_KERNEL };
struct GemmPick {
    GemmFamily family;
    int bm, bn;
    int wm;
    bool f8, lnf;
    int S;
    GemmReduce reduce;
    int launches;
};
GemmPick gemm_pick(const GemmArgs& a, const GemmArgs* b = nullptr);
constexpr int SK_FIXUP_MAX_S = 4;
constexpr int SK_COUNTERS = 8192;
#ifdef LDX_SK_FIXUP_BUILD
inline size_t gemm_sk_ws_floats(int M, int N, int S) { return (size_t)S * ((size_t)M + 255) * ((size_t)N + 255); }
#else
inline size_t gemm_sk_ws_floats(int M, int N, int S) { return (size_t)S * (size_t)M * (size_t)N; }
#endif
bool gemm_sk_fixup(const GemmArgs& a);
void launch_gemm_pp(const GemmArgs& a, int bn, bool lnf, int S, DType dt, hipStream_t s);
void launch_gemm_pp2(const GemmArgs& a, const GemmArgs& b, int bn, DType dt, hipStream_t s);

struct MxQuantArgs { const void* X; int ldx; int rows, K; void* Y; int ldy; uint32_t* S; int s_ld; };
void launch_mx_quant(const MxQuantArgs& a, DType dt, hipStream_t s);

struct SkinnyArgs {
    const float* x; int ldx; const void* W; const float* bias; float* out; int ldo;
    int M, N, K; int in_act; int out_act;
    int accum;
    const void* W8; const uint32_t* SW; int sw_ld;
};
void launch_skinny(const SkinnyArgs& a, DType dt, hipStream_t s);

struct AttnArgs {
    const void* Q; int ldq; const void* K; int ldk; const void* V; int ldv;
    void* O; int ldo;
    int B, H, Nq, Mk, D; float scale; int causal;
    const float* bias; int bias_ld; long bias_hs;
    void* O8; int ldo8; uint32_t* SO; int so_ld;
    float* knorm_ws;
    float* split_ws; int nsplit;
};
void launch_attention(const AttnArgs& a, DType dt, hipStream_t s);
enum AttnFamily : int { AF_ATTN = 0, AF_ATTN32, AF_ATTN32AP, AF_ATTN32G, AF_ATTN40P, AF_ATTN128P, AF_ATTN512 };
struct AttnPick {
    AttnFamily family;
    int targ[3];
    bool kpf;
    int qb, block;
    unsigned grid; int lds;
    bool knorm;
    float thr;
    int nsplit;
    int nsplit_want;
    bool mx_out;
    int launches;
};
AttnPick attn_pick(const AttnArgs& a);
bool attn_pipe_ok(const AttnArgs& a);
void reload_dispatch_env();

constexpr int ATTN40P_LDS = 2 * 64 * (144 + 192), ATTN128P_LDS = 3 * 64 * (272 + 320);
constexpr int ATTN512_QB = 128, ATTN512_KV = 32, ATTN512_LDS = 2 * ATTN512_KV * ((512 * 2 + 16) + (512 * 2 + 64));
void launch_attn_pipe(const AttnArgs& a, const AttnPick& p, DType dt, hipStream_t s);
void launch_attn_pipe128(const AttnArgs& a, const AttnPick& p, DType dt, hipStream_t s);
void launch_attn512(const AttnArgs& a, const AttnPick& p, DType dt, hipStream_t s);
size_t attn512_ws_floats(const AttnArgs& a, int nsplit);
void launch_attn_knorm(const AttnArgs& a, DType dt, hipStream_t s);

struct XAttnArgs {
    void* H; int ldh; long M; int N, C, heads;
    const float* ln_g; const float* ln_b; float eps;
    const void* Wq; const void* Wo; const float* bo;
    const void* K; int ldk; const void* V; int ldv; int Mk;
    float scale;
};
struct FFBlockArgs {
    void* H; int ldh; long M; int C, inner;
    const float* ln_g; const float* ln_b; float eps;
    const void* W1; const float* b1; const void* W2; const float* b2;
};
bool ff_block_ok(const FFBlockArgs& a);
void launch_ff_block(const FFBlockArgs& a, DType dt, hipStream_t s);
struct RowGemmArgs {
    const void* X; int ldx; void* Y; int ldy; long M; int N, K;
    const void* W; const float* bias; const void* R; int ldr;
    int pro; const float* g; const float* b; float eps;
    const float* partial; int nchunk, HW, G;
    float* gn_out; int gn_nchunk;
    int abl;
    long dup_rows;
};
bool rowgemm_ok(const RowGemmArgs& a);
void launch_rowgemm(const RowGemmArgs& a, DType dt, hipStream_t s);
bool xattn_block_ok(const XAttnArgs& a);
void launch_xattn_block(const XAttnArgs& a, DType dt, hipStream_t s);

struct GroupNormArgs {
    const void* X; int ldx; void* Y; int ldy;
    int B, HW, C, G; float eps; int silu;
    const float* gamma; const float* beta;
    float* partial;
    int nchunk;
    int stats_chunks;
};
constexpr int GN_NCHUNK = 256;
constexpr int GN_FOLD = 64;
constexpr int GN_MAX_PRODUCER_CHUNKS = 32768;
static inline size_t gn_workspace_rows(long HWmax) { long r = HWmax / 64; if (r < GN_NCHUNK) r = GN_NCHUNK; if (r > GN_MAX_PRODUCER_CHUNKS) r = GN_MAX_PRODUCER_CHUNKS; return (size_t)r; }
void launch_groupnorm(const GroupNormArgs& a, DType dt, hipStream_t s);
bool gn_uses_small_kernel(int B, long HW, int C, int G);

struct LayerNormArgs {
    const void* X; int ldx; void* Y; int ldy; int rows, C; float eps;
    const float* gamma; const float* beta;
    const float* scale; const float* shift; int mod_ld; int rows_per_batch;
    int rms;
    void* Y8; int ldy8; uint32_t* S8; int s8_ld;
};
void launch_layernorm(const LayerNormArgs& a, DType dt, hipStream_t s);

struct PrepArgs {
    const float* x; const float* sigma; int B, C, H, W; int Cpad; void* xc;
    const float* log_sigmas; int n_sigmas; const float* temb_table; int temb_dim;
    float* temb_out; float* t_out;
    int scale_input;
    const float* t_in;
    int xB;
    const float* cc; int Cx;
    const float* emb_table; int emb_n; float* emb_out;
};
void launch_prep(const PrepArgs& a, DType dt, hipStream_t s);
void launch_timestep(const float* sigma, const float* log_sigmas, int n_sigmas, int n, int* out, hipStream_t s);
struct FinishArgs { const float* eps; int ld; const float* x; const float* sigma; float* out; int B, C, HW; int xB; };
void launch_fill_f32(float* dst, float v, int n, hipStream_t s);
void launch_fill2_f32(float* a, float va, float* b, float vb, int n, hipStream_t s);
void launch_dup_rows(const void* src, void* dst, int rows, int C, int ld, DType dt, hipStream_t s);
void launch_clip_pooled(const float* last, const int* ids, int B, int T, int E, int eos_id, const float* proj, float* out, hipStream_t s);
void launch_finish(const FinishArgs& a, hipStream_t s);

void launch_f32_to_t(const float* in, void* out, size_t n, DType dt, hipStream_t s);
void launch_t_to_f32(const void* in, float* out, size_t n, DType dt, hipStream_t s);
void launch_nchw_to_nhwc(const float* in, void* out, int B, int C, int HW, int Cpad, float scale, DType dt, hipStream_t s);

// ... 51 lines not shown
```

### lightdiffusion-next_amd/csrc/rowblock_store.h

```cpp
#pragma once
#include "ldx_device.h"

namespace ldx {

constexpr int RB_SROW = 320 * 2 + 16;
constexpr int RB_STAGE_BYTES = 64 * RB_SROW;

template <typename T, int QT>
__device__ __forceinline__ void rb_store_rows(T* __restrict__ Y, const int ldy, const long m0, const long M, const int col0, const int wave, const int l15,
                                              const int g4, const int tid, const uint2 (&out)[3][QT], char* sS, const long dup_rows = 0) {
    int tid_ = tid, l15_ = l15;
    asm volatile("" : "+v"(tid_), "+v"(l15_));
#pragma unroll
    for (int hh = 0; hh < QT / 4; ++hh) {
#pragma unroll
        for (int t = 0; t < 3; ++t) {
            const int nl = 16 * t + 4 * g4;
            if (nl < 40) {
#pragma unroll
                for (int q4 = 0; q4 < 4; ++q4) *(uint2*)(sS + (16 * q4 + l15_) * RB_SROW + (wave * 40 + nl) * 2) = out[t][4 * hh + q4];
            }
        }
        __syncthreads();
#pragma unroll
        for (int j = 0; j < 5; ++j) {
            const int idx = tid_ + 512 * j, row = idx / 40, ch = idx - row * 40;
            const long m = m0 + 64 * hh + row;
            if (m < M) {
                const uint4 v = *(const uint4*)(sS + row * RB_SROW + ch * 16);
                *(uint4*)(Y + m * ldy + col0 + ch * 8) = v;
                if (dup_rows) *(uint4*)(Y + (m + dup_rows) * ldy + col0 + ch * 8) = v;
            }
        }
        __syncthreads();
    }
}

}
```

### lightdiffusion-next_amd/csrc/rowgemm.hip

```cpp
#include <hip/hip_runtime.h>
#include <stdint.h>
#include <stdlib.h>
#include "ldx_device.h"
#include "ldx_kernels.h"
#include "rowblock_store.h"

namespace ldx {

template <int CC> struct RgGeom {
    static constexpr int BM = 128 * 320 / CC, QT = BM / 16, LPR = 512 / BM, NH = CC / 320;
    static constexpr int AROW = CC * 2 + 16, ABYTES = BM * AROW;
    static constexpr int TAB = 2 * CC * 4 + 8 * 64 * 4 + 64 * 4;
    static constexpr int LDS = ABYTES + TAB + RB_STAGE_BYTES;
};

template <typename T, int PRO, int CC>
__global__ __launch_bounds__(512, 1) void rowgemm_kernel(const RowGemmArgs p) {
    using G = RgGeom<CC>;
    constexpr int RG_C = CC, RG_BM = G::BM, RG_AROW = G::AROW, RG_ABYTES = G::ABYTES, QT = G::QT, LPR = G::LPR;
    extern __shared__ __attribute__((aligned(16))) char smem[];
    using V8 = typename Vec<T>::v8;
    char* sA = smem;
    float* sSc = (float*)(smem + RG_ABYTES);
    float* sSh = sSc + RG_C;
    float* sRed = sSh + RG_C;
    float* sMR = sRed + 8 * 64;
    const int tid = threadIdx.x, lane = tid & 63;
    const int wave = __builtin_amdgcn_readfirstlane(tid >> 6);
    const int l15_0 = lane & 15, g4_0 = lane >> 4;
    const long m0 = (long)blockIdx.x * RG_BM;
    const T* __restrict__ Xp = (const T*)p.X;
    const T* __restrict__ W = (const T*)p.W;

    const int nown = p.N / G::NH;
    const int npass = nown / 320;
    constexpr int NKS = RG_C / 32, PD = 3;
    uint4 wf[PD + 1][3];
    auto wload = [&](int wrow0_, int l15_, int g4_, int ks, int slot) __attribute__((always_inline)) {
#pragma unroll
        for (int t = 0; t < 3; ++t) {
            const int r = 16 * t + l15_;
            wf[slot][t] = (r < 40) ? *(const uint4*)(W + (long)(wrow0_ + r) * RG_C + ks * 32 + g4_ * 8) : make_uint4(0, 0, 0, 0);
        }
    };
#pragma unroll
    for (int ks = 0; ks < PD; ++ks) wload((int)blockIdx.y * nown + wave * 40, l15_0, g4_0, ks, ks);

    if (PRO == 1) { for (int i = tid; i < RG_C; i += 512) { sSc[i] = p.g[i]; sSh[i] = p.b[i]; } }
    if (PRO == 2) {
        const int b = (int)(m0 / p.HW);
        const int g = tid & 31, st = (tid >> 5) & 1, sl = tid >> 6;
        float a = 0.f;
        {
            const float* pp = p.partial + ((long)b * p.nchunk) * p.G * 2 + g * 2 + st;
            int ck = sl;
            for (; ck + 56 < p.nchunk; ck += 64) {
                float v[8];
#pragma unroll
                for (int u = 0; u < 8; ++u) v[u] = pp[(long)(ck + 8 * u) * p.G * 2];
#pragma unroll
                for (int u = 0; u < 8; ++u) a += v[u];
            }
            for (; ck < p.nchunk; ck += 8) a += pp[(long)ck * p.G * 2];
        }
        sRed[sl * 64 + g * 2 + st] = a;
        __syncthreads();
        if (tid < 32) {
            float su = 0.f, sq = 0.f;
#pragma unroll
            for (int s8 = 0; s8 < 8; ++s8) { su += sRed[s8 * 64 + tid * 2]; sq += sRed[s8 * 64 + tid * 2 + 1]; }
            const float n = (float)p.HW * (float)(RG_C / 32);
            const float mean = su / n;
            const float var = fmaxf(sq / n - mean * mean, 0.f);
            sMR[tid] = mean; sMR[32 + tid] = rsqrtf(var + p.eps);
        }
        __syncthreads();
        for (int c = tid; c < RG_C; c += 512) {
            const int g2 = c / (RG_C / 32);
            const float a2 = sMR[32 + g2] * p.g[c];
            sSc[c] = a2; sSh[c] = p.b[c] - sMR[g2] * a2;
        }
    }
    {
        const int row = tid / LPR, part = tid % LPR;
        const long m = m0 + row;
        uint4 raw[10];
#pragma unroll
        for (int j = 0; j < 10; ++j) raw[j] = (m < p.M && !(p.abl & 4)) ? *(const uint4*)(Xp + m * p.ldx + (part + LPR * j) * 8) : make_uint4(0, 0, 0, 0);
        if (PRO == 0) {
#pragma unroll
            for (int j = 0; j < 10; ++j) *(uint4*)(sA + row * RG_AROW + (part + LPR * j) * 16) = raw[j];
        } else {
            float x[80];
#pragma unroll
            for (int j = 0; j < 10; ++j) {
                float f[8];
                unpack8<T>(raw[j], f);
#pragma unroll
                for (int e = 0; e < 8; ++e) x[8 * j + e] = f[e];
            }
            float mean = 0.f, rstd = 1.f;
            if (PRO == 1) {
                float su = 0.f;
#pragma unroll
                for (int e = 0; e < 80; ++e) su += x[e];
                su += dpp_f<0xB1>(su); su += dpp_f<0x4E>(su); if (LPR == 8) su += dpp_f<0x141>(su);
                mean = su * (1.0f / RG_C);
                float sq = 0.f;
#pragma unroll
                for (int e = 0; e < 80; ++e) { const float d = x[e] - mean; sq = fmaf(d, d, sq); }
                sq += dpp_f<0xB1>(sq); sq += dpp_f<0x4E>(sq); if (LPR == 8) sq += dpp_f<0x141>(sq);
                rstd = rsqrtf(sq * (1.0f / RG_C) + p.eps);
            }
            __syncthreads();
#pragma unroll
            for (int j = 0; j < 10; ++j) {
                const int c0 = (part + LPR * j) * 8;
                float f[8];
#pragma unroll
                for (int e = 0; e < 8; ++e)
                    f[e] = (PRO == 1) ? fmaf((x[8 * j + e] - mean) * rstd, sSc[c0 + e], sSh[c0 + e]) : fmaf(x[8 * j + e], sSc[c0 + e], sSh[c0 + e]);
                *(uint4*)(sA + row * RG_AROW + c0 * 2) = pack8<T>(f);
            }
        }
    }
    __syncthreads();

#pragma unroll 1
    for (int pass = 0; pass < npass; ++pass) {
        int l15 = l15_0, g4 = g4_0;
        asm volatile("" : "+v"(l15), "+v"(g4));
        const int wrow0 = (int)blockIdx.y * nown + pass * 320 + wave * 40;
        f32x4 acc[3][QT];
#pragma unroll
        for (int t = 0; t < 3; ++t)
#pragma unroll
            for (int qt = 0; qt < QT; ++qt) acc[t][qt] = (f32x4){0.f, 0.f, 0.f, 0.f};
        if (!(p.abl & 2))
#pragma unroll
        for (int ks = 0; ks < NKS; ++ks) {
            if (ks + PD < NKS) wload(wrow0, l15, g4, ks + PD, (ks + PD) % (PD + 1));
            V8 af[QT];
#pragma unroll
            for (int qt = 0; qt < QT; ++qt) af[qt] = as_v8<T>(*(const uint4*)(sA + (16 * qt + l15) * RG_AROW + (ks * 32 + g4 * 8) * 2));
#pragma unroll
            for (int t = 0; t < 3; ++t) {
                const V8 w8 = as_v8<T>(wf[ks % (PD + 1)][t]);
#pragma unroll
                for (int qt = 0; qt < QT; ++qt) acc[t][qt] = mfma16(w8, af[qt], acc[t][qt]);
            }
            __builtin_amdgcn_sched_barrier(0);
        }
        __builtin_amdgcn_sched_barrier(0);
        uint2 rr[3][QT];
#pragma unroll
        for (int t = 0; t < 3; ++t)
#pragma unroll
            for (int qt = 0; qt < QT; ++qt) {
                const long m = m0 + 16 * qt + l15;
                const int nl = 16 * t + 4 * g4;
                rr[t][qt] = (p.R && m < p.M && nl < 40 && !(p.abl & 1)) ? *(const uint2*)((const T*)p.R + m * p.ldr + wrow0 + nl) : make_uint2(0u, 0u);
            }
#pragma unroll
        for (int t = 0; t < 3; ++t) {
            const int nl = 16 * t + 4 * g4;
            const int n = wrow0 + (nl < 40 ? nl : 0);
            const float4 bo = p.bias ? *(const float4*)(p.bias + n) : make_float4(0.f, 0.f, 0.f, 0.f);
#pragma unroll
            for (int qt = 0; qt < QT; ++qt) {
                float r4[4];
                unpack4<T>(rr[t][qt], r4);
                rr[t][qt] = pack4<T>(acc[t][qt][0] + bo.x + r4[0], acc[t][qt][1] + bo.y + r4[1], acc[t][qt][2] + bo.z + r4[2], acc[t][qt][3] + bo.w + r4[3]);
            }
        }
        if (p.gn_out) {
            float cs[3][4], cq[3][4];
#pragma unroll
            for (int t = 0; t < 3; ++t) {
#pragma unroll
                for (int r = 0; r < 4; ++r) { cs[t][r] = 0.f; cq[t][r] = 0.f; }
#pragma unroll
                for (int qt = 0; qt < QT; ++qt) {
                    float v4[4];
                    unpack4<T>(rr[t][qt], v4);
#pragma unroll
                    for (int r = 0; r < 4; ++r) { cs[t][r] += v4[r]; cq[t][r] = fmaf(v4[r], v4[r], cq[t][r]); }
                }
#pragma unroll
                for (int r = 0; r < 4; ++r) { cs[t][r] = row16_sum(cs[t][r]); cq[t][r] = row16_sum(cq[t][r]); }
                const int nl = 16 * t + 4 * g4;
                if (l15 == 0 && nl < 40) {
#pragma unroll
                    for (int r = 0; r < 4; ++r) { sSc[(wave * 40 + nl + r) * 2] = cs[t][r]; sSc[(wave * 40 + nl + r) * 2 + 1] = cq[t][r]; }
                }
            }
            __syncthreads();
            const int cpg = p.N / 32;
            if (tid < (320 / cpg) * 2) {
                const int gl = tid >> 1, st = tid & 1;
                float a = 0.f;
                for (int c = 0; c < cpg; ++c) a += sSc[(gl * cpg + c) * 2 + st];
                const int bimg = (int)(m0 / p.HW), chunk = (int)((m0 - (long)bimg * p.HW) / RG_BM);
                const int g0 = ((int)blockIdx.y * nown + pass * 320) / cpg;
                p.gn_out[(((long)bimg * p.gn_nchunk + chunk) * 32 + g0 + gl) * 2 + st] = a;
            }
        }
        if (pass + 1 < npass) {
#pragma unroll
            for (int ks = 0; ks < PD; ++ks) wload(wrow0 + 320, l15, g4, ks, ks);
        }
        if (!(p.abl & 8)) rb_store_rows<T, QT>((T*)p.Y, p.ldy, m0, p.M, (int)blockIdx.y * nown + pass * 320, wave, l15, g4, tid, rr, smem + RG_ABYTES + G::TAB, p.dup_rows);
    }
}

bool rowgemm_ok(const RowGemmArgs& a) {
    static const bool off = getenv("LDX_ROWGEMM") && atoi(getenv("LDX_ROWGEMM")) == 0;
    static const bool off640 = getenv("LDX_ROWGEMM640") && atoi(getenv("LDX_ROWGEMM640")) == 0;
    if (off || (a.K != 320 && a.K != 640) || (a.K == 640 && off640) || a.N <= 0 || a.N % a.K || a.M <= 0 || a.ldx % 8 || a.ldy % 8 || (a.R && a.ldr % 4) || a.pro < 0 || a.pro > 2) return false;
    const int bm = 128 * 320 / a.K;
    if (a.pro >= 1 && (!a.g || !a.b)) return false;
    if (a.pro == 2 && (!a.partial || a.G != 32 || a.HW % bm || a.M % a.HW || a.nchunk < 1 || a.nchunk > GN_NCHUNK)) return false;
    return true;
}
template <typename T, int PRO, int CC>
static void launch_rowgemm_inst(const RowGemmArgs& a, hipStream_t s) {
    using G = RgGeom<CC>;
    static DevOnce once;
    set_dyn_lds(once, (const void*)rowgemm_kernel<T, PRO, CC>, G::LDS);
    hipLaunchKernelGGL((rowgemm_kernel<T, PRO, CC>), dim3((unsigned)((a.M + G::BM - 1) / G::BM), G::NH), dim3(512), G::LDS, s, a);
}
template <typename T>
static void launch_rowgemm_t(const RowGemmArgs& a, hipStream_t s) {
    if (a.K == 320) {
        if (a.pro == 0) launch_rowgemm_inst<T, 0, 320>(a, s); else if (a.pro == 1) launch_rowgemm_inst<T, 1, 320>(a, s); else launch_rowgemm_inst<T, 2, 320>(a, s);
    } else {
        if (a.pro == 0) launch_rowgemm_inst<T, 0, 640>(a, s); else if (a.pro == 1) launch_rowgemm_inst<T, 1, 640>(a, s); else launch_rowgemm_inst<T, 2, 640>(a, s);
    }
}
void launch_rowgemm(const RowGemmArgs& a0, DType dt, hipStream_t s) {
    static const int abl = getenv("LDX_RG_ABL") ? atoi(getenv("LDX_RG_ABL")) : 0;
    RowGemmArgs a = a0; a.abl = abl;
    if (dt == DT_BF16) launch_rowgemm_t<__bf16>(a, s); else launch_rowgemm_t<_Float16>(a, s);
}

}
```

### lightdiffusion-next_amd/csrc/xattn_block.hip

```cpp
#include <hip/hip_runtime.h>
#include <stdint.h>
#include <stdlib.h>
#include "ldx_device.h"
#include "ldx_kernels.h"
#include "rowblock_store.h"

namespace ldx {

namespace {
typedef __attribute__((ext_vector_type(4))) short xs16x4;
__device__ __forceinline__ uint2 x_lds_read_tr16(const char* p) {
    const xs16x4 v = __builtin_amdgcn_ds_read_tr16_b64_v4i16((__attribute__((address_space(3))) xs16x4*)p);
    union { xs16x4 v; uint2 u; } x; x.v = v; return x.u;
}
__device__ __forceinline__ float x_quad_max(float v) {
    auto a = __builtin_amdgcn_permlane16_swap(__float_as_uint(v), __float_as_uint(v), false, false);
    v = fmaxf(__uint_as_float(a[0]), __uint_as_float(a[1]));
    auto b = __builtin_amdgcn_permlane32_swap(__float_as_uint(v), __float_as_uint(v), false, false);
    return fmaxf(__uint_as_float(b[0]), __uint_as_float(b[1]));
}
__device__ __forceinline__ float x_quad_sum(float v) {
    auto a = __builtin_amdgcn_permlane16_swap(__float_as_uint(v), __float_as_uint(v), false, false);
    v = __uint_as_float(a[0]) + __uint_as_float(a[1]);
    auto b = __builtin_amdgcn_permlane32_swap(__float_as_uint(v), __float_as_uint(v), false, false);
    return __uint_as_float(b[0]) + __uint_as_float(b[1]);
}
}

#ifdef XA_ABLATE
__device__ int xa_dbg = 0;
#define XA_DBG(bit) (xa_dbg & (bit))
#else
#define XA_DBG(bit) false
#endif
constexpr int XA_C = 320, XA_H = 8, XA_D = 40, XA_BM = 128, XA_MK = 80;
constexpr int XA_AROW = XA_C * 2 + 16;
constexpr int XA_VROW = 96;
constexpr int XA_ABYTES = XA_BM * XA_AROW, XA_VBYTES = XA_MK * XA_VROW;
constexpr int XA_LDS = XA_ABYTES + XA_H * XA_VBYTES + 2 * XA_C * 4;

template <typename T>
__device__ __forceinline__ void xa_project(const T* __restrict__ W, const int wrow0, const char* sA, const int l15, const int g4, f32x4 (&acc)[3][8]) {
    using V8 = typename Vec<T>::v8;
    constexpr int NKS = XA_C / 32, PD = 3;
#pragma unroll
    for (int t = 0; t < 3; ++t)
#pragma unroll
        for (int qt = 0; qt < 8; ++qt) acc[t][qt] = (f32x4){0.f, 0.f, 0.f, 0.f};
    uint4 wf[PD + 1][3];
    auto wload = [&](int ks, int slot) __attribute__((always_inline)) {
#pragma unroll
        for (int t = 0; t < 3; ++t) {
            const int r = 16 * t + l15;
            uint4 u = make_uint4(0, 0, 0, 0);
            if (r < XA_D) u = *(const uint4*)(W + (long)(wrow0 + r) * XA_C + ks * 32 + g4 * 8);
            wf[slot][t] = u;
        }
    };
#pragma unroll
    for (int ks = 0; ks < PD; ++ks) wload(ks, ks);
#pragma unroll
    for (int ks = 0; ks < NKS; ++ks) {
        if (ks + PD < NKS) wload(ks + PD, (ks + PD) % (PD + 1));
        V8 af[8];
#pragma unroll
        for (int qt = 0; qt < 8; ++qt) af[qt] = as_v8<T>(*(const uint4*)(sA + (16 * qt + l15) * XA_AROW + (ks * 32 + g4 * 8) * 2));
#pragma unroll
        for (int t = 0; t < 3; ++t) {
            const V8 w8 = as_v8<T>(wf[ks % (PD + 1)][t]);
#pragma unroll
            for (int qt = 0; qt < 8; ++qt) acc[t][qt] = mfma16(w8, af[qt], acc[t][qt]);
        }
    }
}

template <typename T>
__global__ __launch_bounds__(512, 1) void xattn_block_kernel(const XAttnArgs p) {
    extern __shared__ __attribute__((aligned(16))) char smem[];
    using V8 = typename Vec<T>::v8;
    char* sA = smem;
    float* sG = (float*)(smem + XA_ABYTES + XA_H * XA_VBYTES);
    float* sBt = sG + XA_C;
    const int tid = threadIdx.x, lane = tid & 63;
    const int wave = __builtin_amdgcn_readfirstlane(tid >> 6);
    const int l15 = lane & 15, g4 = lane >> 4;
    char* sV = smem + XA_ABYTES + wave * XA_VBYTES;
    const long m0 = (long)blockIdx.x * XA_BM;
    const int b = (int)(m0 / p.N);
    T* __restrict__ Hp = (T*)p.H;

    for (int i = tid; i < XA_C; i += 512) { sG[i] = p.ln_g[i]; sBt[i] = p.ln_b[i]; }
    {
        const T* __restrict__ Vp = (const T*)p.V + (long)b * p.Mk * p.ldv + wave * XA_D;
        for (int i = lane; i < XA_VBYTES / 16; i += 64) {
            const int row = i / 6, ch = i - row * 6;
            uint4 u = make_uint4(0, 0, 0, 0);
            if (row < p.Mk && ch < 5) u = *(const uint4*)(Vp + (long)row * p.ldv + ch * 8);
            *(uint4*)(sV + row * XA_VROW + ch * 16) = u;
        }
    }
    {
        const int row = tid >> 2, part = tid & 3;
        const long m = m0 + row;
        float x[80];
        if (m < p.M && !XA_DBG(16)) {
#pragma unroll
            for (int j = 0; j < 10; ++j) {
                const uint4 u = *(const uint4*)(Hp + m * p.ldh + (part + 4 * j) * 8);
                float f[8];
                unpack8<T>(u, f);
#pragma unroll
                for (int e = 0; e < 8; ++e) x[8 * j + e] = f[e];
            }
        } else {
#pragma unroll
            for (int e = 0; e < 80; ++e) x[e] = 0.f;
        }
        float su = 0.f;
#pragma unroll
        for (int e = 0; e < 80; ++e) su += x[e];
        su += dpp_f<0xB1>(su); su += dpp_f<0x4E>(su);
        const float mean = su * (1.0f / XA_C);
        float sq = 0.f;
#pragma unroll
        for (int e = 0; e < 80; ++e) { const float d = x[e] - mean; sq = fmaf(d, d, sq); }
        sq += dpp_f<0xB1>(sq); sq += dpp_f<0x4E>(sq);
        const float rstd = rsqrtf(sq * (1.0f / XA_C) + p.eps);
// ... 153 lines not shown
```

### lightdiffusion-next_amd/engine.py

```python
import ctypes as C
import math

import numbers

import torch

from . import lib
from .weights import T5Config
from .weights import UNetConfig, VAEConfig, CLIPConfig, FluxConfig


def sd15_sigmas():
    betas = torch.linspace(0.00085 ** 0.5, 0.012 ** 0.5, 1000, dtype=torch.float64) ** 2
    alphas_cumprod = torch.cumprod(1.0 - betas, dim=0)
    sigmas = ((1 - alphas_cumprod) / alphas_cumprod) ** 0.5
    return sigmas.float(), sigmas.log().float()


def timestep_index(log_sigmas: torch.Tensor, sigma) -> torch.Tensor:
    sg = torch.as_tensor(sigma, dtype=torch.float32, device="cpu").reshape(-1)
    log_sigma = sg.double().log().float()
    return (log_sigma - log_sigmas[:, None]).abs().argmin(dim=0)


# ... 111 lines not shown
        return out

    def denoise(self, x, sigma, ctx, out=None, c_concat=None, ctx_cached=False):
        if c_concat is None:
            t_idx = self.timestep_index(sigma) if (torch.is_tensor(sigma) and not sigma.is_cuda) else None
            return self._run(self._lib.ldx_unet_denoise, x, sigma, ctx, out, ctx_cached, t_idx=t_idx)
        self._ctx_mode(ctx_cached)
        assert x.is_cuda and x.dtype == torch.float32 and x.dim() == 4, "x must be a CUDA fp32 NCHW tensor"
        b2, ch, h, w = x.shape
        cc = c_concat.to(device=x.device, dtype=torch.float32).contiguous()
        assert cc.dim() == 4 and cc.shape[0] == b2 and cc.shape[2:] == x.shape[2:] and ch + cc.shape[1] == self.cfg.in_channels, "c_concat must be [B2, in_channels - C(x), h, w]"
        x = x.contiguous()
        s = sigma.to(device=x.device, dtype=torch.float32).contiguous()
        ctx = self._ctx_arg(ctx, x.device, ctx_cached)
        assert s.numel() == b2 and ctx.dim() == 3 and ctx.shape[0] == b2 and ctx.shape[2] == self.cfg.context_dim
        if out is None:
            out = torch.empty((b2, self.cfg.out_channels, h, w), device=x.device, dtype=torch.float32)
        lib.check(self._lib.ldx_unet_denoise_concat(self._h, lib.ptr(x), lib.ptr(s), lib.ptr(ctx), lib.ptr(cc), cc.shape[1], b2, h, w, ctx.shape[1],
                                                    lib.ptr(out), lib.current_stream_ptr()), "ldx_unet_denoise_concat")
        return out

    def denoise_cfg(self, x, sigma: float, ctx, out=None, ctx_cached=False):
        self._ctx_mode(ctx_cached)
        assert x.is_cuda and x.dtype == torch.float32 and x.dim() == 4 and x.is_contiguous(), "x must be a contiguous CUDA fp32 NCHW tensor"
        b, ch, h, w = x.shape
        assert ch == self.cfg.in_channels
        assert ctx.is_cuda and ctx.dtype == torch.float32 and ctx.is_contiguous() and ctx.dim() == 3 and ctx.shape[0] == 2 * b and ctx.shape[2] == self.cfg.context_dim
        if out is None:
            out = torch.empty((2 * b, self.cfg.out_channels, h, w), device=x.device, dtype=torch.float32)
        t_index = int(self.timestep_index(float(sigma))[0])
        lib.check(self._lib.ldx_unet_denoise_cfg_t(self._h, lib.ptr(x), float(sigma), t_index, lib.ptr(ctx), b, h, w, ctx.shape[1], lib.ptr(out),
                                                   lib.current_stream_ptr()), "ldx_unet_denoise_cfg_t")
        return out

    def forward(self, x, timesteps, ctx, out=None):
        return self._run(self._lib.ldx_unet_forward, x, timesteps, ctx, out)

    def profile(self, on: bool, reset: bool = True):
        lib.check(self._lib.ldx_profile(self._h, int(on), int(reset)), "ldx_profile")

    def profile_report(self) -> dict:
        import json
        buf = C.create_string_buffer(1 << 18)
        lib.check(self._lib.ldx_profile_report(self._h, buf, len(buf)), "ldx_profile_report")
        return json.loads(buf.value.decode())

    def plan_info(self):
        n, f, a = C.c_int64(), C.c_double(), C.c_int64()
        lib.check(self._lib.ldx_plan_info(self._h, C.byref(n), C.byref(f), C.byref(a)), "ldx_plan_info")
        ex, sh = C.c_double(), C.c_double()
        lib.check(self._lib.ldx_plan_flops(self._h, C.byref(ex), C.byref(sh)), "ldx_plan_flops")
        return {"launches": n.value, "flops": f.value, "arena_bytes": a.value, "flops_executed": ex.value, "flops_shared": sh.value}

    def set_cfg_share(self, mode=True):
        lib.check(self._lib.ldx_unet_cfg_share(self._h, int(mode)), "ldx_unet_cfg_share")


def _load_state_dict(L, h, state_dict, strip=()):
    for k, t in state_dict.items():
        for pre in strip:
            if k.startswith(pre):
                k = k[len(pre):]
        t = t.detach().to("cpu").contiguous()
        if t.dtype not in (torch.float16, torch.bfloat16, torch.float32):
            t = t.float()
        shape = (C.c_int64 * t.dim())(*t.shape)
        lib.check(L.ldx_load_tensor(h, k.encode(), lib.ptr(t), lib.torch_dtype_code(t.dtype), shape, t.dim()),
                  f"ldx_load_tensor({k})")


class VAEDecoderEngine:

    def __init__(self, cfg: VAEConfig, state_dict, device: int = 0, dtype: str = "bf16"):
        self._lib = lib.load()
        self._h = C.c_void_p()
        self.cfg, self.device = cfg, torch.device("cuda", device)
        c = lib.ldx_vae_config()
        c.compute_dtype = {"bf16": lib.LDX_BF16, "f16": lib.LDX_F16, "fp16": lib.LDX_F16}[dtype]
        c.z_channels, c.ch, c.num_levels = cfg.z_channels, cfg.ch, len(cfg.ch_mult)
        for i, v in enumerate(cfg.ch_mult):
            c.ch_mult[i] = v
        c.num_res_blocks, c.out_ch, c.use_post_quant = cfg.num_res_blocks, cfg.out_ch, int(cfg.use_post_quant)
        lib.check(self._lib.ldx_vae_create(C.byref(c), device, C.byref(self._h)), "ldx_vae_create")
        _load_state_dict(self._lib, self._h, state_dict, strip=("first_stage_model.",))
        lib.check(self._lib.ldx_finalize(self._h), "ldx_finalize")

    def decode(self, z):
        assert z.is_cuda and z.dtype == torch.float32 and z.dim() == 4
        b, _, h, w = z.shape
        out = torch.empty((b, 8 * h, 8 * w, self.cfg.out_ch), device=z.device, dtype=torch.float32)
        lib.check(self._lib.ldx_vae_decode(self._h, lib.ptr(z.contiguous()), b, h, w, lib.ptr(out), lib.current_stream_ptr()),
                  "ldx_vae_decode")
        return out

    def encode_moments(self, pixels):
        assert pixels.is_cuda and pixels.dtype == torch.float32 and pixels.dim() == 4 and pixels.shape[-1] == 3
        b, h, w, _ = pixels.shape
        f = 2 ** (len(self.cfg.ch_mult) - 1)
        out = torch.empty((b, 2 * self.cfg.z_channels, h // f, w // f), device=pixels.device, dtype=torch.float32)
        lib.check(self._lib.ldx_vae_encode(self._h, lib.ptr(pixels.contiguous()), b, h, w, lib.ptr(out), lib.current_stream_ptr()),
                  "ldx_vae_encode")
        return out

    def encode(self, pixels):
        mom = self.encode_moments(pixels[..., :3].to(self.device, torch.float32))
        mean, logvar = torch.chunk(mom, 2, dim=1)
# ... 332 lines not shown
```

### lightdiffusion-next_amd/lib.py

```python
import ctypes as C
import os

_HERE = os.path.dirname(os.path.abspath(__file__))
LIB_PATH = os.path.join(_HERE, "libldx.so")

LDX_BF16, LDX_F16, LDX_F32 = 0, 1, 2


class LdxError(RuntimeError):
    pass


class ldx_unet_config(C.Structure):
    _fields_ = [
        ("compute_dtype", C.c_int32),
        ("in_channels", C.c_int32),
        ("out_channels", C.c_int32),
        ("model_channels", C.c_int32),
        ("num_levels", C.c_int32),
        ("channel_mult", C.c_int32 * 8),
        ("num_res_blocks", C.c_int32 * 8),
        ("transformer_depth", C.c_int32 * 32),
        ("transformer_depth_output", C.c_int32 * 48),
        ("transformer_depth_middle", C.c_int32),
        ("num_heads", C.c_int32),
        ("context_dim", C.c_int32),
    ]


class ldx_vae_config(C.Structure):
    _fields_ = [("compute_dtype", C.c_int32), ("z_channels", C.c_int32), ("ch", C.c_int32), ("num_levels", C.c_int32),
                ("ch_mult", C.c_int32 * 8), ("num_res_blocks", C.c_int32), ("out_ch", C.c_int32), ("use_post_quant", C.c_int32)]


class ldx_clip_config(C.Structure):
    _fields_ = [("compute_dtype", C.c_int32), ("hidden_size", C.c_int32), ("num_layers", C.c_int32), ("num_heads", C.c_int32),
                ("intermediate_size", C.c_int32), ("max_positions", C.c_int32), ("vocab_size", C.c_int32)]


class ldx_esrgan_config(C.Structure):
    _fields_ = [("compute_dtype", C.c_int32), ("in_nc", C.c_int32), ("out_nc", C.c_int32), ("nf", C.c_int32), ("gc", C.c_int32),
                ("num_blocks", C.c_int32), ("num_upscale", C.c_int32)]


class ldx_t5_config(C.Structure):
    _fields_ = [("compute_dtype", C.c_int32), ("d_model", C.c_int32), ("d_ff", C.c_int32), ("num_layers", C.c_int32),
                ("num_heads", C.c_int32), ("vocab_size", C.c_int32)]


class ldx_flux_config(C.Structure):
    _fields_ = [("compute_dtype", C.c_int32), ("in_channels", C.c_int32), ("vec_in_dim", C.c_int32), ("context_in_dim", C.c_int32),
                ("hidden_size", C.c_int32), ("mlp_hidden", C.c_int32), ("num_heads", C.c_int32), ("depth", C.c_int32),
                ("depth_single", C.c_int32), ("guidance_embed", C.c_int32)]


_vp, _i, _f, _i64 = C.c_void_p, C.c_int, C.c_float, C.c_int64
_SIGS = {
    "ldx_version": (C.c_char_p, []),
    "ldx_last_error": (C.c_char_p, []),
    "ldx_create": (_i, [C.POINTER(ldx_unet_config), _i, C.POINTER(_vp)]),
    "ldx_destroy": (None, [_vp]),
    "ldx_load_tensor": (_i, [_vp, C.c_char_p, _vp, _i, C.POINTER(_i64), _i]),
    "ldx_set_tables": (_i, [_vp, _vp, _i, _vp, _i]),
    "ldx_finalize": (_i, [_vp]),
    "ldx_unet_denoise": (_i, [_vp, _vp, _vp, _vp, _i, _i, _i, _i, _vp, _vp]),
    "ldx_unet_denoise_cfg": (_i, [_vp, _vp, C.c_float, _vp, _i, _i, _i, _i, _vp, _vp]),
    "ldx_unet_denoise_cfg_t": (_i, [_vp, _vp, C.c_float, _i, _vp, _i, _i, _i, _i, _vp, _vp]),
    "ldx_unet_denoise_t": (_i, [_vp, _vp, _vp, _vp, _vp, _i, _i, _i, _i, _vp, _vp]),
    "ldx_unet_timestep": (_i, [_vp, _vp, _i, _vp, _vp]),
    "ldx_unet_denoise_concat": (_i, [_vp, _vp, _vp, _vp, _vp, _i, _i, _i, _i, _i, _vp, _vp]),
    "ldx_unet_context_cache": (_i, [_vp, _i]),
    "ldx_unet_cfg_share": (_i, [_vp, _i]),
    "ldx_plan_flops": (_i, [_vp, C.POINTER(C.c_double), C.POINTER(C.c_double)]),
    "ldx_reload_env": (_i, []),
    "ldx_unet_forward": (_i, [_vp, _vp, _vp, _vp, _i, _i, _i, _i, _vp, _vp]),
    "ldx_plan_info": (_i, [_vp, C.POINTER(_i64), C.POINTER(C.c_double), C.POINTER(_i64)]),
    "ldx_profile": (_i, [_vp, _i, _i]),
    "ldx_profile_report": (_i, [_vp, C.c_char_p, _i64]),
    "ldx_set_graph_mode": (_i, [_vp, _i]),
    "ldx_graph_stats": (_i, [_vp, C.POINTER(_i64), C.POINTER(_i64)]),
    "ldx_vae_create": (_i, [C.POINTER(ldx_vae_config), _i, C.POINTER(_vp)]),
    "ldx_vae_decode": (_i, [_vp, _vp, _i, _i, _i, _vp, _vp]),
    "ldx_clip_create": (_i, [C.POINTER(ldx_clip_config), _i, C.POINTER(_vp)]),
    "ldx_clip_encode": (_i, [_vp, _vp, _i, _i, _i, _vp, _vp, _vp]),
    "ldx_clip_pooled": (_i, [_vp, _vp, _vp, _i, _i, _i, _vp, _vp]),
    "ldx_clip_set_extra_embeddings": (_i, [_vp, _vp, _i]),
    "ldx_flux_fbcache": (_i, [_vp, _f]),
    "ldx_flux_set_fp8": (_i, [_vp, _i]),
    "ldx_flux_fbcache_stats": (_i, [_vp, C.POINTER(_i64), C.POINTER(_i64)]),
    "ldx_esrgan_create": (_i, [C.POINTER(ldx_esrgan_config), _i, C.POINTER(_vp)]),
    "ldx_esrgan_forward": (_i, [_vp, _vp, _i, _i, _i, _vp, _vp]),
    "ldx_tile_blend": (_i, [_vp, _i, _i, _vp, _vp, _i, _i, _i, _i, _i, _i, _vp]),
    "ldx_tile_finish": (_i, [_vp, _vp, _i64, _i, _vp]),
    "ldx_t5_create": (_i, [C.POINTER(ldx_t5_config), _i, C.POINTER(_vp)]),
    "ldx_t5_encode": (_i, [_vp, _vp, _i, _i, _vp, _vp, _vp]),
    "ldx_flux_create": (_i, [C.POINTER(ldx_flux_config), _i, C.POINTER(_vp)]),
    "ldx_flux_forward": (_i, [_vp, _vp, _vp, _vp, _vp, _vp, _vp, _vp, _i, _i, _i, _i, _i, _vp, _vp]),
    "ldx_sampler_step": (_i, [_i, _vp, _vp, _vp, _vp, _i64, _f, _f, _f, _vp]),
    "ldx_bislerp_pass": (_i, [_vp, _vp, _i, _i, _i, _i, _i, _i, _vp, _vp, _vp, _vp]),
    "ldx_vae_encode": (_i, [_vp, _vp, _i, _i, _i, _vp, _vp]),
    "ldx_bilinear": (_i, [_vp, _vp, _i, _i, _i, _i, _i, _vp]),
    "ldx_op_convert": (_i, [_vp, _vp, _i64, _i, _i, _vp]),
    "ldx_op_gemm": (_i, [_vp, _i, _vp, _i, _i, _i, _vp, _vp, _i, _i, _i, _vp, _i, _vp, _i, _vp, _i, _i, _vp]),
    "ldx_op_conv3x3": (_i, [_vp, _i, _vp, _i, _i, _i, _i, _i, _i, _i, _i, _i, _vp, _vp, _i, _vp, _i, _vp, _i, _i, _vp]),
    "ldx_op_groupnorm": (_i, [_vp, _i, _vp, _i, _i, _i, _i, _i, _f, _i, _vp, _vp, _vp, _i, _vp]),
    "ldx_op_groupnorm_workspace_floats": (_i64, [_i, _i]),
    "ldx_op_conv3x3_skip": (_i, [_vp, _i, _vp, _i, _i, _vp, _i, _i, _i, _i, _i, _vp, _vp, _i, _i, _vp]),
    "ldx_op_layernorm_mx": (_i, [_vp, _i, _i, _i, _f, _vp, _vp, _vp, _i, _vp, _i, _i, _vp]),
    "ldx_op_attention_mx": (_i, [_vp, _i, _vp, _i, _vp, _i, _vp, _i, _vp, _i, _i, _i, _i, _i, _f, _i, _vp]),
    "ldx_op_qk_norm_rope_mx": (_i, [_vp, _i, _i, _i, _i, _vp, _vp, _vp, _vp, _f, _vp, _vp, _i, _vp, _vp, _i, _i, _vp]),
    "ldx_op_mx_vt_quant": (_i, [_vp, _i, _i, _i, _i, _vp, _vp, _i, _i, _vp]),
    "ldx_op_attention_fp8": (_i, [_vp, _i, _vp, _i, _vp, _i, _vp, _i, _vp, _vp, _i, _vp, _i, _vp, _i, _vp, _i, _i, _i, _i, _i, _f, _i, _vp]),
    "ldx_op_mx_quant": (_i, [_vp, _i, _i, _i, _vp, _i, _vp, _i, _i, _vp]),
    "ldx_op_gemm2": (_i, [_vp, _i, _vp, _i, _i, _i, _vp, _vp, _i, _vp, _i, _vp, _i, _i, _i, _vp, _vp, _i, _i, _vp]),
    "ldx_op_gemm2_mx": (_i, [_vp, _i, _vp, _i, _vp, _vp, _i, _i, _i, _i, _vp, _vp, _i, _vp, _i, _vp, _i, _vp, _vp, _i, _i, _i, _i, _vp, _vp, _i, _i, _vp]),
    "ldx_op_gemm_pick": (_i, [_i] * 21 + [C.POINTER(C.c_int32)]),
    "ldx_op_attn_pick": (_i, [_i] * 13 + [C.POINTER(C.c_int32)]),
    "ldx_op_gemm_mx": (_i, [_vp, _i, _vp, _i, _vp, _vp, _i, _i, _i, _i, _vp, _i, _vp, _i, _vp, _i, _vp, _i, _vp, _i, _vp, _i, _i, _vp]),
    "ldx_op_layernorm": (_i, [_vp, _i, _vp, _i, _i, _i, _f, _vp, _vp, _i, _vp]),
    "ldx_op_attention": (_i, [_vp, _i, _vp, _i, _vp, _i, _vp, _i, _i, _i, _i, _i, _i, _f, _i, _i, _vp]),
    "ldx_op_xattn_block": (_i, [_vp, _i, _i64, _i, _i, _i, _vp, _vp, _f, _vp, _vp, _vp, _vp, _i, _vp, _i, _i, _f, _i, _vp]),
    "ldx_op_ff_block": (_i, [_vp, _i, _i64, _i, _i, _vp, _vp, _f, _vp, _vp, _vp, _vp, _i, _vp]),
    "ldx_op_rowgemm": (_i, [_vp, _i, _vp, _i, _i64, _i, _i, _vp, _vp, _vp, _i, _i, _vp, _vp, _f, _vp, _i, _i, _i, _vp]),
    "ldx_op_attention_bias": (_i, [_vp, _i, _vp, _i, _vp, _i, _vp, _i, _i, _i, _i, _i, _i, _f, _vp, _i, _i64, _i, _vp]),
    "ldx_op_skinny": (_i, [_vp, _i, _vp, _vp, _vp, _i, _i, _i, _i, _i, _i, _i, _vp]),
}
EXPORTS = tuple(_SIGS)

_lib = None


def load():
    global _lib
    if _lib is None:
        if not os.path.exists(LIB_PATH):
            raise LdxError(
                f"{LIB_PATH} not found: build it with `python -c 'import __graft_entry__ as g; g.build()'` "
                "(or `make -C lightdiffusion-next_amd/csrc`).  There is no CPU fallback."
            )
        lib = C.CDLL(LIB_PATH)
        for name, (res, args) in _SIGS.items():
            fn = getattr(lib, name)
            fn.restype, fn.argtypes = res, args
        _lib = lib
    return _lib


def check(rc, what=""):
    if rc != 0:
        msg = load().ldx_last_error().decode(errors="replace")
        raise LdxError(f"{what} failed with code {rc}: {msg}")


def ptr(t):
    return None if t is None else C.c_void_p(t.data_ptr())


def torch_dtype_code(dtype):
    import torch

    return {torch.bfloat16: LDX_BF16, torch.float16: LDX_F16, torch.float32: LDX_F32}[dtype]


def current_stream_ptr():
    import torch

    return C.c_void_p(torch.cuda.current_stream().cuda_stream)
```

Measured before the change: 75.22.

## Chain transformer proj_in+LN+QKV, ff_block+proj_out, and fuse key-norm computation

Adds a plan pass that merges the GroupNorm-prologue proj_in rowgemm with the following LayerNorm+QKV rowgemm into one kernel that keeps rows in LDS. It also merges the feed-forward block with the proj_out GEMM and residual add, optionally emitting GroupNorm statistics. The chained rowgemm can compute per-key-block norms for the following attention, so the separate knorm kernel is skipped. This removes launches and intermediate activation round-trips in the 320-channel transformer blocks, at the cost of more complex kernels with higher register and LDS pressure. The chaining is on by default and keyed into the plan cache.

```diff
diff --git a/include/ldx.h b/include/ldx.h
--- a/include/ldx.h
+++ b/include/ldx.h
@@ -109,6 +109,7 @@
                      int B2, int h, int w, int M, float* out_nchw, void* stream);
 int ldx_plan_info(ldx_engine* e, int64_t* n_launches, double* flops, int64_t* arena_bytes);
 int ldx_unet_cfg_share(ldx_engine* e, int enable);
+int ldx_unet_xf_chain(ldx_engine* e, int enable);
 int ldx_plan_flops(ldx_engine* e, double* executed, double* shared);
 int ldx_profile(ldx_engine* e, int enable, int reset);
 int ldx_profile_report(ldx_engine* e, char* buf, int64_t cap);
@@ -196,6 +197,14 @@
                     const void* W1, const float* b1, const void* W2, const float* b2, int dtype, void* stream);
 int ldx_op_rowgemm(const void* X, int ldx, void* Y, int ldy, int64_t M, int N, int K, const void* W, const float* bias, const void* R, int ldr,
                    int pro, const float* gamma, const float* beta, float eps, const float* partial, int nchunk, int HW, int dtype, void* stream);
+int ldx_op_rowgemm_chain(const void* X, int ldx, void* Y, int ldy, int64_t M, int K, const void* W, const float* bias, const float* gamma, const float* beta, float eps,
+                         const float* partial, int nchunk, int HW, const void* W2, const float* bias2, const float* ln_gamma, const float* ln_beta, float ln_eps,
+                         void* Y2, int ldy2, int N2, float* knorm_out, int dtype, void* stream);
+int ldx_op_ff_block_chain(void* H, int ldh, int64_t M, int C, int inner, const float* ln_gamma, const float* ln_beta, float eps,
+                          const void* W1, const float* b1, const void* W2, const float* b2, const void* Wp, const float* bp, const void* X, int ldx,
+                          void* OUT, int ldo, float* gn_out, int HW, int dtype, void* stream);
+int ldx_op_attention_knorm(const void* Q, int ldq, const void* K, int ldk, const void* V, int ldv, void* O, int ldo,
+                           int B, int H, int Nq, int Mk, int D, float scale, float* knorm, int dtype, void* stream);
 int ldx_op_attention_bias(const void* Q, int ldq, const void* K, int ldk, const void* V, int ldv, void* O, int ldo,
                           int B, int H, int Nq, int Mk, int D, float scale, const float* bias, int bias_ld,
                           int64_t bias_head_stride, int dtype, void* stream);
diff --git a/lightdiffusion-next_amd/csrc/attn_pipe.hip b/lightdiffusion-next_amd/csrc/attn_pipe.hip
--- a/lightdiffusion-next_amd/csrc/attn_pipe.hip
+++ b/lightdiffusion-next_amd/csrc/attn_pipe.hip
@@ -337,7 +337,7 @@
 static void launch_attn40p(const AttnArgs& a, const AttnPick& p, hipStream_t s, float thr) {
     if (p.knorm && ABL == 0) {
         const long waves = (long)a.B * a.H * ((a.Mk + 63) / 64);
-        hipLaunchKernelGGL((attn_knorm_kernel<T>), dim3((unsigned)((waves + 3) / 4)), dim3(256), 0, s, a);
+        if (!a.knorm_given) hipLaunchKernelGGL((attn_knorm_kernel<T>), dim3((unsigned)((waves + 3) / 4)), dim3(256), 0, s, a);
         hipLaunchKernelGGL((attn40p_kernel<T, ABL, true>), dim3(p.grid), dim3(p.block), p.lds, s, a, thr);
     } else {
         hipLaunchKernelGGL((attn40p_kernel<T, ABL, false>), dim3(p.grid), dim3(p.block), p.lds, s, a, thr);
diff --git a/lightdiffusion-next_amd/csrc/attn_pipe128.hip b/lightdiffusion-next_amd/csrc/attn_pipe128.hip
--- a/lightdiffusion-next_amd/csrc/attn_pipe128.hip
+++ b/lightdiffusion-next_amd/csrc/attn_pipe128.hip
@@ -347,7 +347,7 @@
 template <typename T, int ABL = 0>
 static void launch_attn128p(const AttnArgs& a, const AttnPick& p, hipStream_t s, float thr) {
     if (p.knorm && ABL == 0) {
-        launch_attn_knorm(a, std::is_same<T, __bf16>::value ? DT_BF16 : DT_F16, s);
+        if (!a.knorm_given) launch_attn_knorm(a, std::is_same<T, __bf16>::value ? DT_BF16 : DT_F16, s);
         static DevOnce once;
         set_dyn_lds(once, (const void*)attn128p_kernel<T, ABL, true>, p.lds);
         hipLaunchKernelGGL((attn128p_kernel<T, ABL, true>), dim3(p.grid), dim3(p.block), p.lds, s, a, thr);
diff --git a/lightdiffusion-next_amd/csrc/capi.cpp b/lightdiffusion-next_amd/csrc/capi.cpp
--- a/lightdiffusion-next_amd/csrc/capi.cpp
+++ b/lightdiffusion-next_amd/csrc/capi.cpp
@@ -299,6 +299,12 @@
     if (!e) { set_error("null engine"); return LDX_EINVAL; }
     if (e->impl->kind != KIND_UNET) { set_error("ldx_unet_cfg_share: not a UNet engine"); return LDX_ESTATE; }
     e->impl->cfg_share = enable < 0 ? 0 : (enable > 2 ? 2 : enable);
+    return LDX_OK;
+}
+int ldx_unet_xf_chain(ldx_engine* e, int enable) {
+    if (!e) { set_error("null engine"); return LDX_EINVAL; }
+    if (e->impl->kind != KIND_UNET) { set_error("ldx_unet_xf_chain: not a UNet engine"); return LDX_ESTATE; }
+    e->impl->xf_chain = enable ? 1 : 0;
     return LDX_OK;
 }
 int ldx_profile(ldx_engine* e, int enable, int reset) {
@@ -611,6 +617,38 @@
     launch_rowgemm(a, dtype_of(dtype), (hipStream_t)stream);
     return check_launch("ldx_op_rowgemm");
 }
+int ldx_op_rowgemm_chain(const void* X, int ldx_, void* Y, int ldy, int64_t M, int K, const void* W, const float* bias, const float* gamma, const float* beta, float eps,
+                         const float* partial, int nchunk, int HW, const void* W2, const float* bias2, const float* ln_gamma, const float* ln_beta, float ln_eps,
+                         void* Y2, int ldy2, int N2, float* knorm_out, int dtype, void* stream) {
+    RowGemmArgs a{};
+    a.X = X; a.ldx = ldx_; a.Y = Y; a.ldy = ldy; a.M = (long)M; a.N = K; a.K = K; a.W = W; a.bias = bias;
+    a.pro = 2; a.g = gamma; a.b = beta; a.eps = eps; a.partial = partial; a.nchunk = nchunk; a.HW = HW; a.G = 32;
+    a.W2 = W2; a.bias2 = bias2; a.g2 = ln_gamma; a.b2 = ln_beta; a.eps2 = ln_eps; a.Y2 = Y2; a.ldy2 = ldy2; a.N2 = N2; a.knorm_out = knorm_out;
+    if (!X || !Y || !W || !W2 || !Y2 || ldx_ < K || ldy < K || HW <= 0 || !rowgemm_ok(a)) {
+        set_error("ldx_op_rowgemm_chain: shape not taken (K = 320, HW % 128 == 0, M % HW == 0, nchunk <= 256, N2 a multiple of 320; key norms: N2 >= 640)"); return LDX_EINVAL; }
+    launch_rowgemm(a, dtype_of(dtype), (hipStream_t)stream);
+    return check_launch("ldx_op_rowgemm_chain");
+}
+int ldx_op_ff_block_chain(void* H, int ldh, int64_t M, int C, int inner, const float* ln_gamma, const float* ln_beta, float eps,
+                          const void* W1, const float* b1, const void* W2, const float* b2, const void* Wp, const float* bp, const void* X, int ldx_,
+                          void* OUT, int ldo, float* gn_out, int HW, int dtype, void* stream) {
+    FFBlockArgs a{};
+    a.H = H; a.ldh = ldh; a.M = (long)M; a.C = C; a.inner = inner; a.ln_g = ln_gamma; a.ln_b = ln_beta; a.eps = eps; a.W1 = W1; a.b1 = b1; a.W2 = W2; a.b2 = b2;
+    a.Wp = Wp; a.bp = bp; a.X = X; a.ldx = ldx_; a.OUT = OUT; a.ldo = ldo; a.gn_out = gn_out; a.HW = HW; a.gn_nchunk = HW > 0 ? HW / 128 : 0;
+    if (!H || !ln_gamma || !ln_beta || !W1 || !b1 || !W2 || !Wp || !X || !OUT || M <= 0 || ldh < C || ldx_ < C || ldo < C || (gn_out && HW <= 0) || !ff_block_ok(a)) {
+        set_error("ldx_op_ff_block_chain: shape not taken by the fused kernel (C = 320, inner = 1280; statistics: HW % 128 == 0, M % HW == 0)"); return LDX_EINVAL; }
+    launch_ff_block(a, dtype_of(dtype), (hipStream_t)stream);
+    return check_launch("ldx_op_ff_block_chain");
+}
+int ldx_op_attention_knorm(const void* Q, int ldq, const void* K, int ldk, const void* V, int ldv, void* O, int ldo, int B, int H, int Nq, int Mk, int D,
+                           float scale, float* knorm, int dtype, void* stream) {
+    if (!Q || !K || !V || !O || !knorm || D % 8 || D <= 0 || ldq % 8 || ldk % 8 || ldv % 8 || ldo % 4 || Mk <= 0) { set_error("ldx_op_attention_knorm: bad argument"); return LDX_EINVAL; }
+    AttnArgs a{Q, ldq, K, ldk, V, ldv, O, ldo, B, H, Nq, Mk, D, scale, 0, nullptr, 0, 0};
+    a.knorm_ws = knorm; a.knorm_given = 1;
+    if (!attn_pipe_ok(a) || !attn_pick(a).knorm) { set_error("ldx_op_attention_knorm: the launch does not go to a pipelined kernel that reads key-block norms"); return LDX_EINVAL; }
+    launch_attention(a, dtype_of(dtype), (hipStream_t)stream);
+    return check_launch("ldx_op_attention_knorm");
+}
 int ldx_op_attention_bias(const void* Q, int ldq, const void* K, int ldk, const void* V, int ldv, void* O, int ldo, int B, int H, int Nq, int Mk, int D,
                           float scale, const float* bias, int bias_ld, int64_t bias_head_stride, int dtype, void* stream) {
     if (!Q || !K || !V || !O || !bias || D % 8 || D > 160 || D <= 0 || ldq % 8 || ldk % 8 || ldv % 8 || ldo % 4 || Mk <= 0 || bias_ld % 4 ||
diff --git a/lightdiffusion-next_amd/csrc/engine.cpp b/lightdiffusion-next_amd/csrc/engine.cpp
--- a/lightdiffusion-next_amd/csrc/engine.cpp
+++ b/lightdiffusion-next_amd/csrc/engine.cpp
@@ -623,6 +623,50 @@
     }
     rowblock_prefix = false;
 }
+void Engine::chain_xf() {
+    const char* tn = dt == DT_BF16 ? "bf16" : "f16";
+    auto merge = [&](size_t i, const Op& o) {
+        Op m = o;
+        m.flops = cur.ops[i].flops + cur.ops[i + 1].flops; m.bytes = cur.ops[i].bytes + cur.ops[i + 1].bytes;
+        cur.ops[i] = m;
+        cur.ops.erase(cur.ops.begin() + (long)i + 1);
+        if (i + 1 < cur.prefix_end) --cur.prefix_end;
+    };
+    for (size_t i = 0; i + 1 < cur.ops.size(); ++i) {
+        const Op& a = cur.ops[i];
+        const Op& b = cur.ops[i + 1];
+        if (a.kind == OP_ROWGEMM && b.kind == OP_ROWGEMM && a.rg.pro == 2 && b.rg.pro == 1 && a.rg.K == 320 && b.rg.K == 320 && b.rg.X == a.rg.Y && b.rg.ldx == a.rg.ldy &&
+            b.rg.M == a.rg.M && !b.rg.R && !a.rg.gn_out && !b.rg.gn_out && !a.rg.dup_rows && !b.rg.dup_rows && (i + 1 < cur.prefix_end) == (i < cur.prefix_end)) {
+            Op o = a;
+            o.rg.W2 = b.rg.W; o.rg.bias2 = b.rg.bias; o.rg.g2 = b.rg.g; o.rg.b2 = b.rg.b; o.rg.eps2 = b.rg.eps; o.rg.Y2 = b.rg.Y; o.rg.ldy2 = b.rg.ldy; o.rg.N2 = b.rg.N;
+            if (!rowgemm_ok(o.rg)) continue;
+            o.name = "xf.proj_in+ln1+qkv";
+            snprintf(o.klabel, sizeof(o.klabel), "rowgemm<%s,2>+ln+qkv", tn);
+            merge(i, o);
+            if (i + 1 < cur.ops.size() && cur.ops[i + 1].kind == OP_ATTN) {
+                RowGemmArgs& r = cur.ops[i].rg;
+                AttnArgs& at = cur.ops[i + 1].at;
+                if (at.knorm_ws && !at.knorm_given && attn_pick(at).knorm && at.K == (const char*)r.Y2 + 320 * 2 && at.ldk == r.ldy2 && at.H == 8 && at.D == 40 && at.Mk == r.HW &&
+                    (long)at.B * at.Mk == r.M && r.N2 >= 640) {
+                    r.knorm_out = at.knorm_ws;
+                    if (rowgemm_ok(r)) { at.knorm_given = 1; snprintf(cur.ops[i].klabel, sizeof(cur.ops[i].klabel), "rowgemm<%s,2>+ln+qkv+knorm", tn); }
+                    else r.knorm_out = nullptr;
+                }
+            }
+            continue;
+        }
+        if (a.kind == OP_FFBLOCK && b.kind == OP_ROWGEMM && b.rg.pro == 0 && b.rg.K == 320 && b.rg.N == 320 && b.rg.X == a.fb.H && b.rg.ldx == a.fb.ldh && b.rg.M == a.fb.M &&
+            b.rg.R && !b.rg.dup_rows && !a.fb.Wp && (i + 1 < cur.prefix_end) == (i < cur.prefix_end)) {
+            Op o = a;
+            o.fb.Wp = b.rg.W; o.fb.bp = b.rg.bias; o.fb.X = b.rg.R; o.fb.ldx = b.rg.ldr; o.fb.OUT = b.rg.Y; o.fb.ldo = b.rg.ldy;
+            o.fb.gn_out = b.rg.gn_out; o.fb.gn_nchunk = b.rg.gn_nchunk; o.fb.HW = b.rg.HW;
+            if (!ff_block_ok(o.fb)) continue;
+            o.name = "xf.ffblock+proj_out";
+            snprintf(o.klabel, sizeof(o.klabel), "ff_block<%s>+proj_out", tn);
+            merge(i, o);
+        }
+    }
+}
 void Engine::op_ln(const char* name, Act X, Act Y, const NormW& n) {
     Op o{}; o.kind = OP_LN; o.name = name;
     LayerNormArgs& l = o.ln;
@@ -813,7 +857,7 @@
 }
 
 int Engine::plan(int B2, int h, int w, int Mc, int share) {
-    return build_plan(PlanKey{B2, h, w, Mc, share}, [&]() -> int {
+    return build_plan(PlanKey{B2, h, w, Mc, share, xf_chain}, [&]() -> int {
         const int mc = cfg.model_channels, ted = 4 * mc;
         const size_t o_temb = a_alloc((size_t)B2 * mc * 4), o_e1 = a_alloc((size_t)B2 * ted * 4), o_e2 = a_alloc((size_t)B2 * ted * 4);
         const size_t o_emb = a_alloc((size_t)B2 * emb_total * 4);
@@ -953,6 +997,7 @@
         }
         fuse_gn_stats();
         fuse_gn_rowgemm();
+        if (xf_chain) chain_xf();
         return LDX_OK;
     });
 }
@@ -1203,7 +1248,7 @@
     if (!x || !sigma_or_t || !ctx || !out || B2 <= 0 || h <= 0 || w <= 0 || Mc <= 0) { set_error("ldx_unet_*: bad argument"); return LDX_EINVAL; }
     HIP_OK(hipSetDevice(device));
     const int share = share_for(B2, h, w, xB, denoise, c_concat != nullptr);
-    if (int rc = select_plan(PlanKey{B2, h, w, Mc, share}, st, [&] { return plan(B2, h, w, Mc, share); })) return rc;
+    if (int rc = select_plan(PlanKey{B2, h, w, Mc, share, xf_chain}, st, [&] { return plan(B2, h, w, Mc, share); })) return rc;
     bind = Bindings{};
     bind.x = x; bind.s = sigma_or_t; bind.ctx = ctx; bind.out = out; bind.den = denoise; bind.xB = xB; bind.cc = c_concat; bind.ccn = cc_channels; bind.t = t_idx;
     bind.ctxc = ctx_cache;
@@ -1264,7 +1309,7 @@
         if (o.kind == OP_GN) n += o.gn.stats_chunks > GN_NCHUNK ? 2 : (o.gn.stats_chunks > 0 ? 1 : 2);
         else if (o.kind == OP_GEMM) n += gemm_pick(o.g).launches;
         else if (o.kind == OP_GEMM2) n += gemm_pick(o.g, &o.g2).launches;
-        else if (o.kind == OP_ATTN) n += attn_pick(o.at).launches;
+        else if (o.kind == OP_ATTN) { const AttnPick ap = attn_pick(o.at); n += ap.launches - (ap.knorm && o.at.knorm_given ? 1 : 0); }
         else n += 1;
     }
     return n;
diff --git a/lightdiffusion-next_amd/csrc/engine.h b/lightdiffusion-next_amd/csrc/engine.h
--- a/lightdiffusion-next_amd/csrc/engine.h
+++ b/lightdiffusion-next_amd/csrc/engine.h
@@ -52,8 +52,8 @@
 struct ProfEntry { long count = 0; double ms = 0, flops = 0, bytes = 0; };
 
 struct PlanKey {
-    int B = 0, h = 0, w = 0, m = 0, share = 0;
-    bool operator==(const PlanKey& o) const { return B == o.B && h == o.h && w == o.w && m == o.m && share == o.share; }
+    int B = 0, h = 0, w = 0, m = 0, share = 0, chain = 0;
+    bool operator==(const PlanKey& o) const { return B == o.B && h == o.h && w == o.w && m == o.m && share == o.share && chain == o.chain; }
     bool operator!=(const PlanKey& o) const { return !(*this == o); }
 };
 
@@ -165,6 +165,7 @@
     int plan(int B2, int h, int w, int Mc, int share = 0);
     int share_for(int B2, int h, int w, int xB, bool denoise, bool concat) const;
     int cfg_share = 1;
+    int xf_chain = 1;
     int64_t n_launches() const;
     int64_t n_graph_captures = 0, n_graph_replays = 0;
     bool profiling = false, prof_detail = false;
@@ -200,6 +201,7 @@
     size_t ws_alloc(size_t bytes);
     void fuse_gn_stats();
     void fuse_gn_rowgemm();
+    void chain_xf();
     bool op_rowgemm(const char* name, Act X, const LinearW& w, Act Y, Act R, int pro, const NormW* nw);
     Bindings bind;
     std::vector<std::vector<ResW>> vae_up; std::vector<LinearW> vae_upconv; std::vector<bool> vae_has_up;
diff --git a/lightdiffusion-next_amd/csrc/ff_block.hip b/lightdiffusion-next_amd/csrc/ff_block.hip
--- a/lightdiffusion-next_amd/csrc/ff_block.hip
+++ b/lightdiffusion-next_amd/csrc/ff_block.hip
@@ -172,12 +172,52 @@
             rr[t][qt] = pack4<T>(y[t][qt][0] + bo.x + r4[0], y[t][qt][1] + bo.y + r4[1], y[t][qt][2] + bo.z + r4[2], y[t][qt][3] + bo.w + r4[3]);
         }
     }
+    if (p.Wp) {
+        rb_rows_to_tile<8>(rr, sA, wave, l15, g4);
+        __syncthreads();
+        int l15_ = l15, g4_ = g4;
+        asm volatile("" : "+v"(l15_), "+v"(g4_));
+        xa_project<T, true>((const T*)p.Wp, wave * 40, sA, l15_, g4_, y);
+        __builtin_amdgcn_sched_barrier(0);
+#pragma unroll
+        for (int t = 0; t < 3; ++t)
+#pragma unroll
+            for (int qt = 0; qt < 8; ++qt) {
+                const long m = m0 + 16 * qt + l15_;
+                const int nl = 16 * t + 4 * g4_;
+                rr[t][qt] = (m < p.M && nl < 40) ? *(const uint2*)((const T*)p.X + m * p.ldx + wave * 40 + nl) : make_uint2(0u, 0u);
+            }
+#pragma unroll
+        for (int t = 0; t < 3; ++t) {
+            const int nl = 16 * t + 4 * g4_;
+            const int n = wave * 40 + (nl < 40 ? nl : 0);
+            const float4 bo = p.bp ? *(const float4*)(p.bp + n) : make_float4(0.f, 0.f, 0.f, 0.f);
+#pragma unroll
+            for (int qt = 0; qt < 8; ++qt) {
+                float r4[4];
+                unpack4<T>(rr[t][qt], r4);
+                rr[t][qt] = pack4<T>(y[t][qt][0] + bo.x + r4[0], y[t][qt][1] + bo.y + r4[1], y[t][qt][2] + bo.z + r4[2], y[t][qt][3] + bo.w + r4[3]);
+            }
+        }
+        if (p.gn_out) {
+            constexpr int QT = 8;
+            const int l15 = l15_, g4 = g4_;
+#define RB_GN_TAB sG
+#define RB_GN_OUT p.gn_out
+#define RB_GN_NCHUNK p.gn_nchunk
+#define RB_GN_HW p.HW
+#define RB_GN_N FB_C
+#define RB_GN_COL0 0
+#include "rowblock_gn.inc"
+        }
+    }
     __syncthreads();
-    rb_store_rows<T, 8>(Hp, p.ldh, m0, p.M, 0, wave, l15, g4, tid, rr, sGb);
+    rb_store_rows<T, 8>(p.Wp ? (T*)p.OUT : Hp, p.Wp ? p.ldo : p.ldh, m0, p.M, 0, wave, l15, g4, tid, rr, sGb);
 }
 
 bool ff_block_ok(const FFBlockArgs& a) {
     static const bool off = getenv("LDX_FF_FUSE") && atoi(getenv("LDX_FF_FUSE")) == 0;
+    if (a.Wp && (!a.X || !a.OUT || a.ldx % 4 || a.ldo % 8 || (a.gn_out && (a.HW <= 0 || a.HW % FB_BM || a.M % a.HW || a.gn_nchunk != a.HW / FB_BM)))) return false;
     return !off && a.C == FB_C && a.inner == FB_I && a.M > 0 && a.ldh % 8 == 0 && a.b1 != nullptr;
 }
 template <typename T>
diff --git a/lightdiffusion-next_amd/csrc/ldx_kernels.h b/lightdiffusion-next_amd/csrc/ldx_kernels.h
--- a/lightdiffusion-next_amd/csrc/ldx_kernels.h
+++ b/lightdiffusion-next_amd/csrc/ldx_kernels.h
@@ -93,6 +93,7 @@
     void* O8; int ldo8; uint32_t* SO; int so_ld;
     float* knorm_ws;
     float* split_ws; int nsplit;
+    int knorm_given;
 };
 void launch_attention(const AttnArgs& a, DType dt, hipStream_t s);
 enum AttnFamily : int { AF_ATTN = 0, AF_ATTN32, AF_ATTN32AP, AF_ATTN32G, AF_ATTN40P, AF_ATTN128P, AF_ATTN512 };
@@ -132,6 +133,7 @@
     void* H; int ldh; long M; int C, inner;
     const float* ln_g; const float* ln_b; float eps;
     const void* W1; const float* b1; const void* W2; const float* b2;
+    const void* Wp; const float* bp; const void* X; int ldx; void* OUT; int ldo; float* gn_out; int gn_nchunk; int HW;
 };
 bool ff_block_ok(const FFBlockArgs& a);
 void launch_ff_block(const FFBlockArgs& a, DType dt, hipStream_t s);
@@ -143,6 +145,8 @@
     float* gn_out; int gn_nchunk;
     int abl;
     long dup_rows;
+    const void* W2; const float* bias2; const float* g2; const float* b2; float eps2; void* Y2; int ldy2; int N2;
+    float* knorm_out;
 };
 bool rowgemm_ok(const RowGemmArgs& a);
 void launch_rowgemm(const RowGemmArgs& a, DType dt, hipStream_t s);
diff --git a/lightdiffusion-next_amd/csrc/rowblock_gn.inc b/lightdiffusion-next_amd/csrc/rowblock_gn.inc
--- /dev/null
+++ b/lightdiffusion-next_amd/csrc/rowblock_gn.inc
@@ -0,0 +1,38 @@
+{
+    float cs[3][4], cq[3][4];
+#pragma unroll
+    for (int t = 0; t < 3; ++t) {
+#pragma unroll
+        for (int r = 0; r < 4; ++r) { cs[t][r] = 0.f; cq[t][r] = 0.f; }
+#pragma unroll
+        for (int qt = 0; qt < QT; ++qt) {
+            float v4[4];
+            unpack4<T>(rr[t][qt], v4);
+#pragma unroll
+            for (int r = 0; r < 4; ++r) { cs[t][r] += v4[r]; cq[t][r] = fmaf(v4[r], v4[r], cq[t][r]); }
+        }
+#pragma unroll
+        for (int r = 0; r < 4; ++r) { cs[t][r] = row16_sum(cs[t][r]); cq[t][r] = row16_sum(cq[t][r]); }
+        const int nl = 16 * t + 4 * g4;
+        if (l15 == 0 && nl < 40) {
+#pragma unroll
+            for (int r = 0; r < 4; ++r) { (RB_GN_TAB)[(wave * 40 + nl + r) * 2] = cs[t][r]; (RB_GN_TAB)[(wave * 40 + nl + r) * 2 + 1] = cq[t][r]; }
+        }
+    }
+    __syncthreads();
+    const int cpg = (RB_GN_N) / 32;
+    if (tid < (320 / cpg) * 2) {
+        const int gl = tid >> 1, st = tid & 1;
+        float a = 0.f;
+        for (int c = 0; c < cpg; ++c) a += (RB_GN_TAB)[(gl * cpg + c) * 2 + st];
+        const int bimg = (int)(m0 / (RB_GN_HW)), chunk = (int)((m0 - (long)bimg * (RB_GN_HW)) / (16 * QT));
+        const int g0 = (RB_GN_COL0) / cpg;
+        (RB_GN_OUT)[(((long)bimg * (RB_GN_NCHUNK) + chunk) * 32 + g0 + gl) * 2 + st] = a;
+    }
+}
+#undef RB_GN_TAB
+#undef RB_GN_OUT
+#undef RB_GN_NCHUNK
+#undef RB_GN_HW
+#undef RB_GN_N
+#undef RB_GN_COL0
diff --git a/lightdiffusion-next_amd/csrc/rowblock_store.h b/lightdiffusion-next_amd/csrc/rowblock_store.h
--- a/lightdiffusion-next_amd/csrc/rowblock_store.h
+++ b/lightdiffusion-next_amd/csrc/rowblock_store.h
@@ -6,7 +6,57 @@
 constexpr int RB_SROW = 320 * 2 + 16;
 constexpr int RB_STAGE_BYTES = 64 * RB_SROW;
 
-template <typename T, int QT>
+constexpr int RB_C = 320, RB_AROW = RB_C * 2 + 16;
+
+template <typename T, bool FENCE = false>
+__device__ __forceinline__ void xa_project(const T* __restrict__ W, const int wrow0, const char* sA, const int l15, const int g4, f32x4 (&acc)[3][8]) {
+    using V8 = typename Vec<T>::v8;
+    constexpr int NKS = RB_C / 32, PD = 3;
+#pragma unroll
+    for (int t = 0; t < 3; ++t)
+#pragma unroll
+        for (int qt = 0; qt < 8; ++qt) acc[t][qt] = (f32x4){0.f, 0.f, 0.f, 0.f};
+    uint4 wf[PD + 1][3];
+    auto wload = [&](int ks, int slot) __attribute__((always_inline)) {
+#pragma unroll
+        for (int t = 0; t < 3; ++t) {
+            const int r = 16 * t + l15;
+            uint4 u = make_uint4(0, 0, 0, 0);
+            if (r < 40) u = *(const uint4*)(W + (long)(wrow0 + r) * RB_C + ks * 32 + g4 * 8);
+            wf[slot][t] = u;
+        }
+    };
+#pragma unroll
+    for (int ks = 0; ks < PD; ++ks) wload(ks, ks);
+#pragma unroll
+    for (int ks = 0; ks < NKS; ++ks) {
+        if (ks + PD < NKS) wload(ks + PD, (ks + PD) % (PD + 1));
+        V8 af[8];
+#pragma unroll
+        for (int qt = 0; qt < 8; ++qt) af[qt] = as_v8<T>(*(const uint4*)(sA + (16 * qt + l15) * RB_AROW + (ks * 32 + g4 * 8) * 2));
+#pragma unroll
+        for (int t = 0; t < 3; ++t) {
+            const V8 w8 = as_v8<T>(wf[ks % (PD + 1)][t]);
+#pragma unroll
+            for (int qt = 0; qt < 8; ++qt) acc[t][qt] = mfma16(w8, af[qt], acc[t][qt]);
+        }
+        if (FENCE) __builtin_amdgcn_sched_barrier(0);
+    }
+}
+
+template <int QT>
+__device__ __forceinline__ void rb_rows_to_tile(const uint2 (&out)[3][QT], char* sA, const int wave, const int l15, const int g4) {
+#pragma unroll
+    for (int t = 0; t < 3; ++t) {
+        const int nl = 16 * t + 4 * g4;
+        if (nl < 40) {
+#pragma unroll
+            for (int qt = 0; qt < QT; ++qt) *(uint2*)(sA + (16 * qt + l15) * RB_AROW + (wave * 40 + nl) * 2) = out[t][qt];
+        }
+    }
+}
+
+template <typename T, int QT, bool FULL = false>
 __device__ __forceinline__ void rb_store_rows(T* __restrict__ Y, const int ldy, const long m0, const long M, const int col0, const int wave, const int l15,
                                               const int g4, const int tid, const uint2 (&out)[3][QT], char* sS, const long dup_rows = 0) {
     int tid_ = tid, l15_ = l15;
@@ -26,7 +76,7 @@
         for (int j = 0; j < 5; ++j) {
             const int idx = tid_ + 512 * j, row = idx / 40, ch = idx - row * 40;
             const long m = m0 + 64 * hh + row;
-            if (m < M) {
+            if (FULL || m < M) {
                 const uint4 v = *(const uint4*)(sS + row * RB_SROW + ch * 16);
                 *(uint4*)(Y + m * ldy + col0 + ch * 8) = v;
                 if (dup_rows) *(uint4*)(Y + (m + dup_rows) * ldy + col0 + ch * 8) = v;
diff --git a/lightdiffusion-next_amd/csrc/rowgemm.hip b/lightdiffusion-next_amd/csrc/rowgemm.hip
--- a/lightdiffusion-next_amd/csrc/rowgemm.hip
+++ b/lightdiffusion-next_amd/csrc/rowgemm.hip
@@ -1,6 +1,7 @@
 #include <hip/hip_runtime.h>
 #include <stdint.h>
 #include <stdlib.h>
+#include <type_traits>
 #include "ldx_device.h"
 #include "ldx_kernels.h"
 #include "rowblock_store.h"
@@ -14,8 +15,30 @@
     static constexpr int LDS = ABYTES + TAB + RB_STAGE_BYTES;
 };
 
+template <int LPR, int C>
+__device__ __forceinline__ void rg_ln_stats(const float (&x)[80], const float eps, float& mean, float& rstd) {
+    float su = 0.f;
+#pragma unroll
+    for (int e = 0; e < 80; ++e) su += x[e];
+    su += dpp_f<0xB1>(su); su += dpp_f<0x4E>(su); if (LPR == 8) su += dpp_f<0x141>(su);
+    mean = su * (1.0f / C);
+    float sq = 0.f;
+#pragma unroll
+    for (int e = 0; e < 80; ++e) { const float d = x[e] - mean; sq = fmaf(d, d, sq); }
+    sq += dpp_f<0xB1>(sq); sq += dpp_f<0x4E>(sq); if (LPR == 8) sq += dpp_f<0x141>(sq);
+    rstd = rsqrtf(sq * (1.0f / C) + eps);
+}
+__device__ __forceinline__ float rg_quad_sum(float v) {
+    auto a = __builtin_amdgcn_permlane16_swap(__float_as_uint(v), __float_as_uint(v), false, false);
+    v = __uint_as_float(a[0]) + __uint_as_float(a[1]);
+    auto b = __builtin_amdgcn_permlane32_swap(__float_as_uint(v), __float_as_uint(v), false, false);
+    return __uint_as_float(b[0]) + __uint_as_float(b[1]);
+}
+
 template <typename T, int PRO, int CC>
 __global__ __launch_bounds__(512, 1) void rowgemm_kernel(const RowGemmArgs p) {
+    constexpr bool CHAIN = PRO == 2 && CC == 320;
+    constexpr bool FULL = PRO == 2;
     using G = RgGeom<CC>;
     constexpr int RG_C = CC, RG_BM = G::BM, RG_AROW = G::AROW, RG_ABYTES = G::ABYTES, QT = G::QT, LPR = G::LPR;
     extern __shared__ __attribute__((aligned(16))) char smem[];
@@ -29,11 +52,11 @@
     const int wave = __builtin_amdgcn_readfirstlane(tid >> 6);
     const int l15_0 = lane & 15, g4_0 = lane >> 4;
     const long m0 = (long)blockIdx.x * RG_BM;
+    const int by = G::NH == 1 ? 0 : (int)blockIdx.y;
     const T* __restrict__ Xp = (const T*)p.X;
     const T* __restrict__ W = (const T*)p.W;
 
-    const int nown = p.N / G::NH;
-    const int npass = nown / 320;
+    const int nown0 = p.N / G::NH;
     constexpr int NKS = RG_C / 32, PD = 3;
     uint4 wf[PD + 1][3];
     auto wload = [&](int wrow0_, int l15_, int g4_, int ks, int slot) __attribute__((always_inline)) {
@@ -44,7 +67,7 @@
         }
     };
 #pragma unroll
-    for (int ks = 0; ks < PD; ++ks) wload((int)blockIdx.y * nown + wave * 40, l15_0, g4_0, ks, ks);
+    for (int ks = 0; ks < PD; ++ks) wload(by * nown0 + wave * 40, l15_0, g4_0, ks, ks);
 
     if (PRO == 1) { for (int i = tid; i < RG_C; i += 512) { sSc[i] = p.g[i]; sSh[i] = p.b[i]; } }
     if (PRO == 2) {
@@ -86,7 +109,7 @@
         const long m = m0 + row;
         uint4 raw[10];
 #pragma unroll
-        for (int j = 0; j < 10; ++j) raw[j] = (m < p.M && !(p.abl & 4)) ? *(const uint4*)(Xp + m * p.ldx + (part + LPR * j) * 8) : make_uint4(0, 0, 0, 0);
+        for (int j = 0; j < 10; ++j) raw[j] = ((FULL || m < p.M) && !(p.abl & 4)) ? *(const uint4*)(Xp + m * p.ldx + (part + LPR * j) * 8) : make_uint4(0, 0, 0, 0);
         if (PRO == 0) {
 #pragma unroll
             for (int j = 0; j < 10; ++j) *(uint4*)(sA + row * RG_AROW + (part + LPR * j) * 16) = raw[j];
@@ -100,18 +123,7 @@
                 for (int e = 0; e < 8; ++e) x[8 * j + e] = f[e];
             }
             float mean = 0.f, rstd = 1.f;
-            if (PRO == 1) {
-                float su = 0.f;
-#pragma unroll
-                for (int e = 0; e < 80; ++e) su += x[e];
-                su += dpp_f<0xB1>(su); su += dpp_f<0x4E>(su); if (LPR == 8) su += dpp_f<0x141>(su);
-                mean = su * (1.0f / RG_C);
-                float sq = 0.f;
-#pragma unroll
-                for (int e = 0; e < 80; ++e) { const float d = x[e] - mean; sq = fmaf(d, d, sq); }
-                sq += dpp_f<0xB1>(sq); sq += dpp_f<0x4E>(sq); if (LPR == 8) sq += dpp_f<0x141>(sq);
-                rstd = rsqrtf(sq * (1.0f / RG_C) + p.eps);
-            }
+            if (PRO == 1) rg_ln_stats<LPR, RG_C>(x, p.eps, mean, rstd);
             __syncthreads();
 #pragma unroll
             for (int j = 0; j < 10; ++j) {
@@ -126,11 +138,29 @@
     }
     __syncthreads();
 
+    bool chained = false;
+    if constexpr (CHAIN) chained = p.W2 != nullptr;
+    auto late = [&]() __attribute__((always_inline)) {
+        const RowGemmArgs* q = (const RowGemmArgs*)__builtin_amdgcn_kernarg_segment_ptr();
+        return q;
+    };
+    auto parg = [&]() __attribute__((always_inline)) { if constexpr (CHAIN) return late(); else return &p; };
+    auto run_passes = [&](auto S1) __attribute__((always_inline)) {
+    constexpr bool s1 = decltype(S1)::value;
+    const float* const bias = s1 ? late()->bias2 : parg()->bias;
+    const T* const Rp = s1 ? nullptr : (const T*)parg()->R;
+    T* const Yp = (T*)(s1 ? late()->Y2 : parg()->Y);
+    const int ldy = s1 ? late()->ldy2 : parg()->ldy;
+    float* const gn_out = (s1 || PRO == 2) ? nullptr : parg()->gn_out;
+    const long dup_rows = s1 ? 0 : parg()->dup_rows;
+    const int ldr = s1 ? 0 : parg()->ldr;
+    const int nown = s1 ? late()->N2 : nown0;
+    const int npass = nown / 320;
 #pragma unroll 1
     for (int pass = 0; pass < npass; ++pass) {
         int l15 = l15_0, g4 = g4_0;
         asm volatile("" : "+v"(l15), "+v"(g4));
-        const int wrow0 = (int)blockIdx.y * nown + pass * 320 + wave * 40;
+        const int wrow0 = by * nown + pass * 320 + wave * 40;
         f32x4 acc[3][QT];
 #pragma unroll
         for (int t = 0; t < 3; ++t)
@@ -159,13 +189,13 @@
             for (int qt = 0; qt < QT; ++qt) {
                 const long m = m0 + 16 * qt + l15;
                 const int nl = 16 * t + 4 * g4;
-                rr[t][qt] = (p.R && m < p.M && nl < 40 && !(p.abl & 1)) ? *(const uint2*)((const T*)p.R + m * p.ldr + wrow0 + nl) : make_uint2(0u, 0u);
+                rr[t][qt] = (Rp && (FULL || m < p.M) && nl < 40 && !(p.abl & 1)) ? *(const uint2*)(Rp + m * ldr + wrow0 + nl) : make_uint2(0u, 0u);
             }
 #pragma unroll
         for (int t = 0; t < 3; ++t) {
             const int nl = 16 * t + 4 * g4;
             const int n = wrow0 + (nl < 40 ? nl : 0);
-            const float4 bo = p.bias ? *(const float4*)(p.bias + n) : make_float4(0.f, 0.f, 0.f, 0.f);
+            const float4 bo = bias ? *(const float4*)(bias + n) : make_float4(0.f, 0.f, 0.f, 0.f);
 #pragma unroll
             for (int qt = 0; qt < QT; ++qt) {
                 float r4[4];
@@ -173,43 +203,88 @@
                 rr[t][qt] = pack4<T>(acc[t][qt][0] + bo.x + r4[0], acc[t][qt][1] + bo.y + r4[1], acc[t][qt][2] + bo.z + r4[2], acc[t][qt][3] + bo.w + r4[3]);
             }
         }
-        if (p.gn_out) {
-            float cs[3][4], cq[3][4];
-#pragma unroll
-            for (int t = 0; t < 3; ++t) {
-#pragma unroll
-                for (int r = 0; r < 4; ++r) { cs[t][r] = 0.f; cq[t][r] = 0.f; }
+        if (gn_out) {
+#define RB_GN_TAB sSc
+#define RB_GN_OUT gn_out
+#define RB_GN_NCHUNK p.gn_nchunk
+#define RB_GN_HW p.HW
+#define RB_GN_N p.N
+#define RB_GN_COL0 (by * nown + pass * 320)
+#include "rowblock_gn.inc"
+        }
+        if constexpr (CHAIN) {
+            float* const knorm_out = s1 && pass == 1 ? late()->knorm_out : nullptr;
+            if (knorm_out) {
+                float mx[2] = {0.f, 0.f};
 #pragma unroll
                 for (int qt = 0; qt < QT; ++qt) {
-                    float v4[4];
-                    unpack4<T>(rr[t][qt], v4);
-#pragma unroll
-                    for (int r = 0; r < 4; ++r) { cs[t][r] += v4[r]; cq[t][r] = fmaf(v4[r], v4[r], cq[t][r]); }
+                    float ss = 0.f;
+#pragma unroll
+                    for (int t = 0; t < 3; ++t) {
+                        float v4[4];
+                        unpack4<T>(rr[t][qt], v4);
+                        if (16 * t + 4 * g4 < 40) {
+#pragma unroll
+                            for (int r = 0; r < 4; ++r) ss = fmaf(v4[r], v4[r], ss);
+                        }
+                    }
+                    ss = rg_quad_sum(ss);
+                    mx[qt / 4] = fmaxf(mx[qt / 4], ss);
                 }
-#pragma unroll
-                for (int r = 0; r < 4; ++r) { cs[t][r] = row16_sum(cs[t][r]); cq[t][r] = row16_sum(cq[t][r]); }
-                const int nl = 16 * t + 4 * g4;
-                if (l15 == 0 && nl < 40) {
-#pragma unroll
-                    for (int r = 0; r < 4; ++r) { sSc[(wave * 40 + nl + r) * 2] = cs[t][r]; sSc[(wave * 40 + nl + r) * 2 + 1] = cq[t][r]; }
+                mx[0] = row16_max(mx[0]); mx[1] = row16_max(mx[1]);
+                if (lane == 0) {
+                    const int bimg = (int)(m0 / p.HW), nblk = p.HW / 64, blk0 = (int)((m0 - (long)bimg * p.HW) / 64);
+                    float* kn = knorm_out + ((long)bimg * 8 + wave) * nblk + blk0;
+                    kn[0] = sqrtf(mx[0]) * 1.002f; kn[1] = sqrtf(mx[1]) * 1.002f;
                 }
             }
+        }
+        if (pass + 1 < npass) {
+#pragma unroll
+            for (int ks = 0; ks < PD; ++ks) wload(wrow0 + 320, l15, g4, ks, ks);
+        }
+        if constexpr (CHAIN) {
+            if (!s1 && chained) {
+                W = (const T*)late()->W2;
+#pragma unroll
+                for (int ks = 0; ks < PD; ++ks) wload(wave * 40, l15, g4, ks, ks);
+            }
+        }
+        if (!(p.abl & 8)) rb_store_rows<T, QT, FULL>(Yp, ldy, m0, p.M, by * nown + pass * 320, wave, l15, g4, tid, rr, smem + RG_ABYTES + G::TAB, dup_rows);
+        if constexpr (CHAIN) {
+            if (!s1 && chained) rb_rows_to_tile<QT>(rr, sA, wave, l15, g4);
+        }
+    }
+    };
+    run_passes(std::false_type{});
+    if constexpr (CHAIN) {
+        if (chained) {
+            { const RowGemmArgs* q = late(); for (int i = tid; i < RG_C; i += 512) { sSc[i] = q->g2[i]; sSh[i] = q->b2[i]; } }
             __syncthreads();
-            const int cpg = p.N / 32;
-            if (tid < (320 / cpg) * 2) {
-                const int gl = tid >> 1, st = tid & 1;
-                float a = 0.f;
-                for (int c = 0; c < cpg; ++c) a += sSc[(gl * cpg + c) * 2 + st];
-                const int bimg = (int)(m0 / p.HW), chunk = (int)((m0 - (long)bimg * p.HW) / RG_BM);
-                const int g0 = ((int)blockIdx.y * nown + pass * 320) / cpg;
-                p.gn_out[(((long)bimg * p.gn_nchunk + chunk) * 32 + g0 + gl) * 2 + st] = a;
-            }
-        }
-        if (pass + 1 < npass) {
-#pragma unroll
-            for (int ks = 0; ks < PD; ++ks) wload(wrow0 + 320, l15, g4, ks, ks);
-        }
-        if (!(p.abl & 8)) rb_store_rows<T, QT>((T*)p.Y, p.ldy, m0, p.M, (int)blockIdx.y * nown + pass * 320, wave, l15, g4, tid, rr, smem + RG_ABYTES + G::TAB, p.dup_rows);
+            int tid_ = tid;
+            asm volatile("" : "+v"(tid_));
+            const int row = tid_ / LPR, part = tid_ % LPR;
+            float x[80];
+#pragma unroll
+            for (int j = 0; j < 10; ++j) {
+                float f[8];
+                unpack8<T>(*(const uint4*)(sA + row * RG_AROW + (part + LPR * j) * 16), f);
+#pragma unroll
+                for (int e = 0; e < 8; ++e) x[8 * j + e] = f[e];
+            }
+            float mean, rstd;
+            rg_ln_stats<LPR, RG_C>(x, late()->eps2, mean, rstd);
+#pragma unroll
+            for (int j = 0; j < 10; ++j) {
+                const int c0 = (part + LPR * j) * 8;
+                float f[8];
+#pragma unroll
+                for (int e = 0; e < 8; ++e) f[e] = fmaf((x[8 * j + e] - mean) * rstd, sSc[c0 + e], sSh[c0 + e]);
+                *(uint4*)(sA + row * RG_AROW + c0 * 2) = pack8<T>(f);
+            }
+            __syncthreads();
+            run_passes(std::true_type{});
+        }
     }
 }
 
@@ -219,7 +294,12 @@
     if (off || (a.K != 320 && a.K != 640) || (a.K == 640 && off640) || a.N <= 0 || a.N % a.K || a.M <= 0 || a.ldx % 8 || a.ldy % 8 || (a.R && a.ldr % 4) || a.pro < 0 || a.pro > 2) return false;
     const int bm = 128 * 320 / a.K;
     if (a.pro >= 1 && (!a.g || !a.b)) return false;
+    if (a.pro == 2 && a.gn_out) return false;
     if (a.pro == 2 && (!a.partial || a.G != 32 || a.HW % bm || a.M % a.HW || a.nchunk < 1 || a.nchunk > GN_NCHUNK)) return false;
+    if (a.W2) {
+        if (a.pro != 2 || a.K != 320 || a.N != 320 || !a.Y2 || !a.g2 || !a.b2 || a.N2 <= 0 || a.N2 % 320 || a.ldy2 % 8 || a.ldy2 < a.N2 || a.gn_out) return false;
+        if (a.knorm_out && (a.N2 < 640 || a.HW % 128)) return false;
+    } else if (a.knorm_out) return false;
     return true;
 }
 template <typename T, int PRO, int CC>
diff --git a/lightdiffusion-next_amd/csrc/xattn_block.hip b/lightdiffusion-next_amd/csrc/xattn_block.hip
--- a/lightdiffusion-next_amd/csrc/xattn_block.hip
+++ b/lightdiffusion-next_amd/csrc/xattn_block.hip
@@ -34,45 +34,10 @@
 #define XA_DBG(bit) false
 #endif
 constexpr int XA_C = 320, XA_H = 8, XA_D = 40, XA_BM = 128, XA_MK = 80;
-constexpr int XA_AROW = XA_C * 2 + 16;
+constexpr int XA_AROW = RB_AROW;
 constexpr int XA_VROW = 96;
 constexpr int XA_ABYTES = XA_BM * XA_AROW, XA_VBYTES = XA_MK * XA_VROW;
 constexpr int XA_LDS = XA_ABYTES + XA_H * XA_VBYTES + 2 * XA_C * 4;
-
-template <typename T>
-__device__ __forceinline__ void xa_project(const T* __restrict__ W, const int wrow0, const char* sA, const int l15, const int g4, f32x4 (&acc)[3][8]) {
-    using V8 = typename Vec<T>::v8;
-    constexpr int NKS = XA_C / 32, PD = 3;
-#pragma unroll
-    for (int t = 0; t < 3; ++t)
-#pragma unroll
-        for (int qt = 0; qt < 8; ++qt) acc[t][qt] = (f32x4){0.f, 0.f, 0.f, 0.f};
-    uint4 wf[PD + 1][3];
-    auto wload = [&](int ks, int slot) __attribute__((always_inline)) {
-#pragma unroll
-        for (int t = 0; t < 3; ++t) {
-            const int r = 16 * t + l15;
-            uint4 u = make_uint4(0, 0, 0, 0);
-            if (r < XA_D) u = *(const uint4*)(W + (long)(wrow0 + r) * XA_C + ks * 32 + g4 * 8);
-            wf[slot][t] = u;
-        }
-    };
-#pragma unroll
-    for (int ks = 0; ks < PD; ++ks) wload(ks, ks);
-#pragma unroll
-    for (int ks = 0; ks < NKS; ++ks) {
-        if (ks + PD < NKS) wload(ks + PD, (ks + PD) % (PD + 1));
-        V8 af[8];
-#pragma unroll
-        for (int qt = 0; qt < 8; ++qt) af[qt] = as_v8<T>(*(const uint4*)(sA + (16 * qt + l15) * XA_AROW + (ks * 32 + g4 * 8) * 2));
-#pragma unroll
-        for (int t = 0; t < 3; ++t) {
-            const V8 w8 = as_v8<T>(wf[ks % (PD + 1)][t]);
-#pragma unroll
-            for (int qt = 0; qt < 8; ++qt) acc[t][qt] = mfma16(w8, af[qt], acc[t][qt]);
-        }
-    }
-}
 
 template <typename T>
 __global__ __launch_bounds__(512, 1) void xattn_block_kernel(const XAttnArgs p) {
diff --git a/lightdiffusion-next_amd/engine.py b/lightdiffusion-next_amd/engine.py
--- a/lightdiffusion-next_amd/engine.py
+++ b/lightdiffusion-next_amd/engine.py
@@ -187,6 +187,9 @@
         lib.check(self._lib.ldx_plan_flops(self._h, C.byref(ex), C.byref(sh)), "ldx_plan_flops")
         return {"launches": n.value, "flops": f.value, "arena_bytes": a.value, "flops_executed": ex.value, "flops_shared": sh.value}
 
+    def set_xf_chain(self, enable=True):
+        lib.check(self._lib.ldx_unet_xf_chain(self._h, int(bool(enable))), "ldx_unet_xf_chain")
+
     def set_cfg_share(self, mode=True):
         lib.check(self._lib.ldx_unet_cfg_share(self._h, int(mode)), "ldx_unet_cfg_share")
 
diff --git a/lightdiffusion-next_amd/lib.py b/lightdiffusion-next_amd/lib.py
--- a/lightdiffusion-next_amd/lib.py
+++ b/lightdiffusion-next_amd/lib.py
@@ -71,6 +71,7 @@
     "ldx_unet_denoise_concat": (_i, [_vp, _vp, _vp, _vp, _vp, _i, _i, _i, _i, _i, _vp, _vp]),
     "ldx_unet_context_cache": (_i, [_vp, _i]),
     "ldx_unet_cfg_share": (_i, [_vp, _i]),
+    "ldx_unet_xf_chain": (_i, [_vp, _i]),
     "ldx_plan_flops": (_i, [_vp, C.POINTER(C.c_double), C.POINTER(C.c_double)]),
     "ldx_reload_env": (_i, []),
     "ldx_unet_forward": (_i, [_vp, _vp, _vp, _vp, _i, _i, _i, _i, _vp, _vp]),
@@ -122,6 +123,9 @@
     "ldx_op_xattn_block": (_i, [_vp, _i, _i64, _i, _i, _i, _vp, _vp, _f, _vp, _vp, _vp, _vp, _i, _vp, _i, _i, _f, _i, _vp]),
     "ldx_op_ff_block": (_i, [_vp, _i, _i64, _i, _i, _vp, _vp, _f, _vp, _vp, _vp, _vp, _i, _vp]),
     "ldx_op_rowgemm": (_i, [_vp, _i, _vp, _i, _i64, _i, _i, _vp, _vp, _vp, _i, _i, _vp, _vp, _f, _vp, _i, _i, _i, _vp]),
+    "ldx_op_rowgemm_chain": (_i, [_vp, _i, _vp, _i, _i64, _i, _vp, _vp, _vp, _vp, _f, _vp, _i, _i, _vp, _vp, _vp, _vp, _f, _vp, _i, _i, _vp, _i, _vp]),
+    "ldx_op_ff_block_chain": (_i, [_vp, _i, _i64, _i, _i, _vp, _vp, _f, _vp, _vp, _vp, _vp, _vp, _vp, _vp, _i, _vp, _i, _vp, _i, _i, _vp]),
+    "ldx_op_attention_knorm": (_i, [_vp, _i, _vp, _i, _vp, _i, _vp, _i, _i, _i, _i, _i, _i, _f, _vp, _i, _vp]),
     "ldx_op_attention_bias": (_i, [_vp, _i, _vp, _i, _vp, _i, _vp, _i, _i, _i, _i, _i, _i, _f, _vp, _i, _i64, _i, _vp]),
     "ldx_op_skinny": (_i, [_vp, _i, _vp, _vp, _vp, _i, _i, _i, _i, _i, _i, _i, _vp]),
 }
```

Result: no change. 75.69, median of 6 (+0.6%).
